# timoklein/alphazero-gym

Hardware: AMD Instinct MI355X
Metric: MCTS sims/sec (whole node), Pendulum-v1 4096 trees n_sims=200, 1/2/4/8 GPU (higher is better)
Workload: dtype f32; 1 GPU; config C: Pendulum-v1 A0C, 4096 trees/GPU x 200 sims, 2x256 ELU policy/value MLP, c_uct=0.05 c_pw=1 kappa=0.5; trees_per_gpu=4096, n_sims=200, parallelism=1 GPU

## Files before the change

### alphazero_gym_amd/csrc/azg_engine.hip

```cpp
#include <hip/hip_runtime.h>

#include <cmath>
#include <cstdio>
#include <cstdlib>
#include <cstring>
#include <string>
#include <vector>

#include "engine_host.h"
#include "env.cuh"
#include "mlp.cuh"
#include "tree.cuh"
#include "aux_kernels.cuh"


static std::string g_create_err;

static int fail(azg_engine* e, int code, const std::string& msg) {
    if (e) e->err = msg; else g_create_err = msg;
    return code;
}

#define HIPCHK(e, call)                                                                                  \
    do {                                                                                                 \
        hipError_t _rc = (call);                                                                         \
        if (_rc != hipSuccess) return fail(e, AZG_E_DEVICE, std::string(#call) + ": " + hipGetErrorString(_rc)); \
    } while (0)

struct DeviceScope {
    int prev;
    bool ok;
    explicit DeviceScope(int dev) : prev(-1) {
        if (hipGetDevice(&prev) != hipSuccess) prev = -1;
        ok = (prev == dev) || hipSetDevice(dev) == hipSuccess;
        if (prev == dev) prev = -1;
    }
    ~DeviceScope() { if (prev >= 0) (void)hipSetDevice(prev); }
};
#define ON_DEVICE(e)                                     \
    DeviceScope _scope((e)->cfg.device_id);              \
    if (!_scope.ok) return fail(e, AZG_E_DEVICE, "hipSetDevice failed")

template <typename T>
static int dalloc(azg_engine* e, T** p, size_t n, std::vector<void*>& reg) {
    void* q = nullptr;
    hipError_t rc = hipMalloc(&q, n * sizeof(T) > 0 ? n * sizeof(T) : 16);
    if (rc != hipSuccess) return fail(e, AZG_E_DEVICE, std::string("hipMalloc: ") + hipGetErrorString(rc));
    reg.push_back(q);
    *p = (T*)q;
    return AZG_OK;
}

static int ls_prepare(azg_engine* e) {
    if (e->ls_hp == e->HP) return AZG_OK;
    for (void* p : e->ls_allocs) (void)hipFree(p);
    e->ls_allocs.clear();
    const size_t B = e->cfg.n_trees, G = ((B + TREES_PER_WG - 1) / TREES_PER_WG + 3) / 4 * 4, HP = e->HP;
    float* obsT; float *a0, *a1, *parts; LsTree* tr; LsLane* ln;
    e->team_cnt_bytes = (((B + 31) / 32) * 8 * 32 + 32) * sizeof(unsigned);
    if (dalloc(e, &e->d_team_cnt, e->team_cnt_bytes / 4, e->ls_allocs) ||
        dalloc(e, &obsT, G * 64, e->ls_allocs) || dalloc(e, &a0, G * HP * 16, e->ls_allocs) || dalloc(e, &a1, G * HP * 16, e->ls_allocs) ||
        dalloc(e, &parts, G * (HP / 64) * 64 * 4, e->ls_allocs) || dalloc(e, &tr, B, e->ls_allocs) ||
        dalloc(e, &ln, B * 16, e->ls_allocs))
        return AZG_E_DEVICE;
    e->ls.obsT = obsT; e->ls.act[0] = (f32x4*)a0; e->ls.act[1] = (f32x4*)a1; e->ls.parts = (f32x4*)parts;
    e->ls.tree = tr; e->ls.lane = ln;
    if (hipMemset(obsT, 0, G * 64 * sizeof(float)) != hipSuccess || hipMemset(a0, 0, G * HP * 16 * sizeof(float)) != hipSuccess || hipMemset(a1, 0, G * HP * 16 * sizeof(float)) != hipSuccess) return AZG_E_DEVICE;
    e->ls_hp = e->HP;
    return AZG_OK;
}

static size_t stamp_rows(size_t B) {
    size_t r = ((B + 3) / 4) * 4;
    const size_t r8 = ((B + 15) / 16) * 8, team = ((B + 31) / 32) * 16 * 3 / 2;
    if (r8 > r) r = r8;
    if (team > r) r = team;
    return r < 16 ? 16 : r;
}

static int env_digit(const char* name, int dflt) {
    const char* v = getenv(name);
    return (v && v[0] >= '0' && v[0] <= '9') ? v[0] - '0' : dflt;
}

static bool use_lockstep(const azg_engine* e) {
    if (e->opt.force_persistent) return false;
    if (e->P.in8) return false;
    return e->HP >= 512 && e->n_hidden >= 2 && !e->P.layernorm;
}

template <int ENV>
static hipError_t search_path(azg_engine* e, bool lockstep) {
    if (lockstep) {
        if constexpr (ENV == AZG_ENV_ACROBOT) return hipErrorInvalidValue;
        else return azg_lockstep_search<ENV>(e);
    }
    return e->HP <= 128 ? azg_persistent_search<ENV, false>(e) : azg_persistent_search<ENV, true>(e);
}
static hipError_t search_launch(azg_engine* e, bool lockstep) {
    switch (azg_kernel_env(e->cfg)) {
        case AZG_ENV_CARTPOLE: return search_path<AZG_ENV_CARTPOLE>(e, lockstep);
        case AZG_ENV_MOUNTAINCAR_CONT: return search_path<AZG_ENV_MOUNTAINCAR_CONT>(e, lockstep);
        case AZG_ENV_ACROBOT: return search_path<AZG_ENV_ACROBOT>(e, lockstep);
        default: return search_path<AZG_ENV_PENDULUM_V1>(e, lockstep);
    }
}

extern "C" int azg_search_resident(azg_engine* e);
static int team_check(azg_engine* e) {
    if (!e->team_pending) return AZG_OK;
    unsigned flag = 0;
    e->team_pending = 0;
    if (hipMemcpy(&flag, e->d_team_cnt + (e->team_cnt_bytes / 4 - 1), 4, hipMemcpyDeviceToHost) != hipSuccess)
        return fail(e, AZG_E_DEVICE, "reading the team kernel's status failed");
    if (flag) e->opt.ls_team = 0;
    if (flag == 0) return AZG_OK;
    e->team_fallbacks += 1;
    e->search_idx = e->team_search_idx;
    int rc = azg_search_resident(e);
    if (rc) return rc;
    if (hipStreamSynchronize(e->stream) != hipSuccess) return fail(e, AZG_E_DEVICE, "hipStreamSynchronize failed");
    return AZG_OK;
}

extern "C" {

int azg_abi_version(void) { return AZG_ABI_VERSION; }

const char* azg_last_error(const azg_engine* e) { return e ? e->err.c_str() : g_create_err.c_str(); }

void azg_engine_destroy(azg_engine* e) {
    if (!e) return;
    DeviceScope scope(e->cfg.device_id);
    if (e->stream) (void)hipStreamSynchronize(e->stream);
    for (void* p : e->dev_allocs) (void)hipFree(p);
    for (void* p : e->dist_allocs) (void)hipFree(p);
    if (e->d_wblob) (void)hipFree(e->d_wblob);
    if (e->d_wmap) (void)hipFree(e->d_wmap);
    if (e->h_res_block) (void)hipHostFree(e->h_res_block);
    if (e->d_eval) (void)hipFree(e->d_eval);
    for (void* p : e->sp_allocs) (void)hipFree(p);
    for (void* p : e->ls_allocs) (void)hipFree(p);
    if (e->ev0) (void)hipEventDestroy(e->ev0);
    if (e->ev1) (void)hipEventDestroy(e->ev1);
    if (e->stream) (void)hipStreamDestroy(e->stream);
    delete e;
}

static int mapped_hip_runtimes(std::string& paths) {
    static int cached_n = -1;
    static std::string cached_paths;
    if (cached_n >= 0) { paths = cached_paths; return cached_n; }
    std::vector<std::string> seen;
    FILE* f = fopen("/proc/self/maps", "r");
    if (!f) return 0;
    char line[1024];
    while (fgets(line, sizeof line, f)) {
        if (!strstr(line, "libamdhip64")) continue;
        const char* p = strchr(line, '/');
        if (!p) continue;
        std::string path(p);
        while (!path.empty() && (path.back() == '\n' || path.back() == ' ')) path.pop_back();
        bool dup = false;
        for (const auto& q : seen) dup = dup || q == path;
        if (!dup) seen.push_back(path);
    }
    fclose(f);
    paths.clear();
    for (const auto& q : seen) paths += (paths.empty() ? "" : ", ") + q;
    cached_paths = paths;
    cached_n = (int)seen.size();
    return cached_n;
}

int azg_engine_create(const azg_config* cfg, azg_engine** out) {
    if (!cfg || !out) return fail(nullptr, AZG_E_INVALID, "null argument");
    {
        std::string rts;
        const char* allow = getenv("AZG_ALLOW_MULTI_HIP");
        if (mapped_hip_runtimes(rts) > 1 && !(allow && allow[0] == '1'))
            return fail(nullptr, AZG_E_DEVICE, ("two HIP runtimes are mapped in this process (" + rts + "): load PyTorch (import torch) BEFORE "
                                               "libazgym_hip.so so that both use PyTorch's copy; if they are meant to coexist (differing "
                                               "SONAMEs, a deliberate second copy), set AZG_ALLOW_MULTI_HIP=1").c_str());
    }
    if (cfg->struct_size != (int32_t)sizeof(azg_config)) return fail(nullptr, AZG_E_INVALID, "azg_config size mismatch");
    if (cfg->n_trees < 1 || cfg->n_sims < 1) return fail(nullptr, AZG_E_INVALID, "n_trees and n_sims must be >= 1");
    if (cfg->env_id < 0 || cfg->env_id > AZG_ENV_ACROBOT) return fail(nullptr, AZG_E_INVALID, "unknown env_id");
    const bool discrete_env = cfg->env_id == AZG_ENV_CARTPOLE || cfg->env_id == AZG_ENV_MOUNTAINCAR || cfg->env_id == AZG_ENV_ACROBOT;
    if (cfg->mode == AZG_MODE_DISCRETE && !discrete_env)
        return fail(nullptr, AZG_E_UNSUPPORTED, "discrete mode requires a discrete-action env (CartPole, MountainCar, Acrobot)");
    if (cfg->mode == AZG_MODE_CONTINUOUS && discrete_env)
        return fail(nullptr, AZG_E_UNSUPPORTED, "continuous mode requires a continuous-action env (Pendulum, MountainCarContinuous)");
    if (cfg->mode == AZG_MODE_DISCRETE && cfg->num_actions != (cfg->env_id == AZG_ENV_CARTPOLE ? 2 : 3))
        return fail(nullptr, AZG_E_INVALID, "num_actions does not match the env (CartPole 2, MountainCar 3, Acrobot 3)");
    if (cfg->tie_break != AZG_TIE_FIRST && cfg->tie_break != AZG_TIE_RANDOM) return fail(nullptr, AZG_E_INVALID, "unknown tie_break");
    if (cfg->mode == AZG_MODE_CONTINUOUS && !(cfg->c_pw > 0.0 && cfg->c_pw < 1e6 && cfg->kappa >= 0.0 && cfg->kappa <= 8.0))
        return fail(nullptr, AZG_E_INVALID, "c_pw must be > 0 and kappa >= 0 (progressive widening: ceil(c_pw (n + 1)^kappa) children)");
    int ndev = 0;
    if (hipGetDeviceCount(&ndev) != hipSuccess || ndev < 1) return fail(nullptr, AZG_E_DEVICE, "no HIP device available");
    if (cfg->device_id < 0 || cfg->device_id >= ndev) return fail(nullptr, AZG_E_DEVICE, "device_id out of range");
    azg_engine* e = new azg_engine();
    e->cfg = *cfg;
    e->opt.force_persistent = env_digit("AZG_FORCE_PERSISTENT", 0) == 1;
    e->opt.force_stream_weights = env_digit("AZG_FORCE_STREAM_WEIGHTS", 0) == 1;
    e->opt.force_global_tree = env_digit("AZG_FORCE_GLOBAL_TREE", 0) == 1;
    e->opt.no_spec = env_digit("AZG_NO_SPEC", 0) == 1;
    e->opt.waves = env_digit("AZG_WAVES", 0);
    e->opt.groups = env_digit("AZG_GROUPS", 0);
    { const char* v = getenv("AZG_TRACE_CAP"); const int t = v ? atoi(v) : 0; e->opt.trace_cap = t > 0 ? t : 0; }
    { const char* v = getenv("AZG_TILE_TREES"); const int t = v ? atoi(v) : 0; e->opt.tile_trees = (t == 16 || t == 8) ? t : 0; }
    e->opt.ls_team = env_digit("AZG_LS_TEAM", 1);
    e->opt.team_wide = env_digit("AZG_TEAM_WIDE", 1);
    { const char* v = getenv("AZG_TEAM_TT"); e->opt.team_tt = v ? atoi(v) : 0; }
    { const char* v = getenv("AZG_TEAM_SPIN_LIMIT"); e->opt.team_spin_limit = v ? atol(v) : (1L << 23); }
    e->opt.no_lds_state = getenv("AZG_NO_LDS_STATE") != nullptr;
    e->d_team_cnt = nullptr; e->team_cnt_bytes = 0; e->team_pending = 0; e->team_fallbacks = 0; e->team_search_idx = 0;
    e->lds_warned = 0; e->last_search_idx = 0; e->ms_kept = 0.0f; e->ms_kept_valid = 0;
    e->carry_max = 0;
    e->n_nets = 1; e->net_have.assign(1, 0);
    e->h_res_block = nullptr; e->d_res_block = nullptr; e->res_bytes = 0;
    e->d_wblob = nullptr; e->d_wmap = nullptr; e->w_floats = 0; e->dist_nd = -1; e->dist_ncomp = -1;
    e->d_eval = nullptr; e->eval_floats = 0;
    e->stream = nullptr; e->ev0 = e->ev1 = nullptr;
    e->publish_always = env_digit("AZG_PUBLISH_TREES", 0) == 1; e->publish_once = 0; e->published = 0; e->redo_ok = 0;
    e->mlp_ready = 0; e->searched = 0; e->results_valid = 0; e->search_idx = 0; e->last_ms = 0.0f; e->sp_on = 0; e->ls_hp = 0;
    e->S_env = (cfg->env_id == AZG_ENV_CARTPOLE || cfg->env_id == AZG_ENV_ACROBOT) ? 4 : 2;
    e->S_obs = cfg->env_id == AZG_ENV_ACROBOT ? 6 : (cfg->env_id == AZG_ENV_CARTPOLE ? 4 : ((cfg->env_id == AZG_ENV_MOUNTAINCAR || cfg->env_id == AZG_ENV_MOUNTAINCAR_CONT) ? 2 : 3));
    const int ns = cfg->n_sims;
    std::vector<int> pw(ns + 2, 0);
    if (cfg->mode == AZG_MODE_CONTINUOUS) {
        int kmax = 1;
        for (int n = 0; n < ns + 2; ++n) {
            double v = std::ceil(cfg->c_pw * std::pow((double)(n + 1), cfg->kappa));
            if (v > 1e6) v = 1e6;
            pw[n] = (int)v;
            if (n < ns && pw[n] > kmax) kmax = pw[n];
        }
        e->Kmax = kmax;
        e->R = ns + 2;
        e->nd = 2;
    } else {
        e->Kmax = cfg->num_actions;
        e->R = 1 + cfg->num_actions * (ns + 1);
        e->nd = cfg->num_actions;
    }
    if (e->R > 32767) { delete e; return fail(nullptr, AZG_E_UNSUPPORTED, "tree too large: records per tree must be < 32768"); }
    if (cfg->tie_break == AZG_TIE_RANDOM && e->Kmax > 16) { delete e; return fail(nullptr, AZG_E_UNSUPPORTED, "tie_break random supports at most 16 children per node"); }
    e->Kp = (e->Kmax + 15) / 16 * 16;
    e->tab_n = cfg->mode == AZG_MODE_CONTINUOUS ? ns + 2 : 4 * ns + 4;
    DeviceScope scope(cfg->device_id);
    if (!scope.ok) { delete e; return fail(nullptr, AZG_E_DEVICE, "hipSetDevice failed"); }
    e->n_cus = 256;
    (void)hipDeviceGetAttribute(&e->n_cus, hipDeviceAttributeMultiprocessorCount, cfg->device_id);
#define CK(x) do { int _r = (x); if (_r != AZG_OK) { g_create_err = e->err; azg_engine_destroy(e); return _r; } } while (0)
#define HK(call) do { hipError_t _rc = (call); if (_rc != hipSuccess) { g_create_err = std::string(#call) + ": " + hipGetErrorString(_rc); azg_engine_destroy(e); return AZG_E_DEVICE; } } while (0)
    HK(hipStreamCreateWithFlags(&e->stream, hipStreamNonBlocking));
    HK(hipEventCreate(&e->ev0));
    HK(hipEventCreate(&e->ev1));
    KParams& P = e->P;
    memset(&P, 0, sizeof(P));
    const size_t B = (size_t)cfg->n_trees, R = (size_t)e->R;
    RecL* hot; Cold* cold; double* edge_W; float* action; float* prior; unsigned short* child; int* n_rec;
    int* d_pw; double* d_sq;
    CK(dalloc(e, &hot, B * R, e->dev_allocs));
    CK(dalloc(e, &cold, B * R, e->dev_allocs));
    CK(dalloc(e, &edge_W, B * R, e->dev_allocs));
    CK(dalloc(e, &action, B * R, e->dev_allocs));
    CK(dalloc(e, &prior, B * R, e->dev_allocs));
    CK(dalloc(e, &child, B * R * e->Kp, e->dev_allocs));
    CK(dalloc(e, &n_rec, B, e->dev_allocs));
    CK(dalloc(e, &d_pw, (size_t)ns + 2, e->dev_allocs));
    CK(dalloc(e, &d_sq, (size_t)e->tab_n, e->dev_allocs));
    CK(dalloc(e, &e->d_roots, B * e->S_env, e->dev_allocs));
    CK(dalloc(e, &e->d_carry, B, e->dev_allocs));
    const size_t K = (size_t)e->Kmax;
    {
        e->res_bytes = B * K * 8 + B * 8 + B * K * 4 + B * K * 4 + B * 4;
        char* blk;
        CK(dalloc(e, &blk, e->res_bytes, e->dev_allocs));
        e->d_res_block = blk;
        e->d_Q = (double*)blk; e->d_vt = (double*)(blk + B * K * 8);
        e->d_actions = (float*)(blk + B * K * 8 + B * 8); e->d_counts = (int*)(blk + B * K * 8 + B * 8 + B * K * 4);
        e->d_nch = (int*)(blk + B * K * 8 + B * 8 + B * K * 8);
        HK(hipHostMalloc(&e->h_res_block, e->res_bytes, hipHostMallocDefault));
    }
    CK(dalloc(e, &e->d_child_n, B * K, e->dev_allocs));
    CK(dalloc(e, &e->d_child_state, B * K * e->S_env, e->dev_allocs));
    CK(dalloc(e, &e->d_rootV, B, e->dev_allocs));
    CK(dalloc(e, &e->d_rootdist, B * e->nd, e->dev_allocs));
    {
        unsigned long long* st;
        CK(dalloc(e, &st, stamp_rows(B) * 16, e->dev_allocs));
        e->P.stamps = st;
        e->stamp_n = stamp_rows(B);
    }
    std::vector<double> sq(e->tab_n);
    for (int n = 0; n < e->tab_n; ++n) sq[n] = std::sqrt((double)(n + 1));
    HK(hipMemcpy(d_pw, pw.data(), sizeof(int) * (ns + 2), hipMemcpyHostToDevice));
    HK(hipMemcpy(d_sq, sq.data(), sizeof(double) * e->tab_n, hipMemcpyHostToDevice));
    HK(hipMemset(hot, 0, B * R * sizeof(RecL)));
    HK(hipMemset(e->d_carry, 0, B * sizeof(int)));
    P.B = cfg->n_trees; P.n_sims = ns; P.R = e->R; P.Kp = e->Kp; P.A = cfg->num_actions; P.nd = e->nd;
    P.trace_cap = e->opt.trace_cap > 0 ? e->opt.trace_cap : 5;
    P.tie_random = cfg->tie_break == AZG_TIE_RANDOM; P.env_id = cfg->env_id; P.v1 = cfg->env_id == AZG_ENV_PENDULUM_V1; P.tree_base = cfg->tree_id_base; P.mode = cfg->mode;
    P.c_uct = cfg->c_uct; P.gamma = cfg->gamma; P.epsilon = cfg->epsilon; P.reward_scale = cfg->reward_scale;
    P.c_uct_f = (float)cfg->c_uct; P.gamma_f = (float)cfg->gamma; P.bound_f = (float)cfg->action_bound;
    P.seed = cfg->seed; P.S = e->S_env; P.tab_n = e->tab_n; P.pw0 = cfg->mode == AZG_MODE_CONTINUOUS ? pw[0] : 0;
    P.roots = e->d_roots; P.carry = e->d_carry;
    P.hot = hot; P.cold = cold; P.edge_W = edge_W; P.action = action; P.prior = prior; P.child = child;
    P.n_rec = n_rec; P.pw_need = d_pw; P.sqrt_tab = d_sq;
    P.res_actions = e->d_actions; P.res_counts = e->d_counts; P.res_Q = e->d_Q; P.res_vt = e->d_vt; P.res_nch = e->d_nch;
    P.res_child_n = e->d_child_n; P.res_child_state = e->d_child_state; P.res_root_V = e->d_rootV; P.res_root_dist = e->d_rootdist;
    P.res_Kmax = e->Kmax; P.res_v_target = cfg->v_target;
    P.net_T = cfg->n_trees; P.net_wgs = 1; P.net_wstride = 0;
    *out = e;
    return AZG_OK;
#undef CK
#undef HK
}

static int pad64(int n) { return (n + 63) / 64 * 64; }
static inline int unit_of(int i) { int t = i >> 4, r = (i >> 2) & 3, g = i & 3; return 16 * t + 4 * g + r; }

static bool same_desc(const azg_mlp_desc& a, const azg_mlp_desc& b) {
    if (a.in_dim != b.in_dim || a.n_hidden != b.n_hidden || a.n_dist != b.n_dist || a.layernorm != b.layernorm) return false;
    for (int l = 0; l < a.n_hidden; ++l) if (a.hidden[l] != b.hidden[l]) return false;
    return true;
}

static int check_desc(azg_engine* e, const azg_mlp_desc* d, size_t n_floats, int* HP_out, int* ncomp_out) {
    if (d->struct_size != (int32_t)sizeof(azg_mlp_desc)) return fail(e, AZG_E_INVALID, "azg_mlp_desc size mismatch");
    if (d->n_hidden < 1 || d->n_hidden > AZG_MAX_HIDDEN_LAYERS) return fail(e, AZG_E_INVALID, "n_hidden out of range");
    if (d->activation < 0 || d->activation > AZG_ACT_HARDSWISH) return fail(e, AZG_E_INVALID, "unknown activation");
    if (d->in_dim != e->S_obs) return fail(e, AZG_E_INVALID, "in_dim does not match the env observation");
    int ncomp = 0;
    if (e->cfg.mode == AZG_MODE_CONTINUOUS) {
        ncomp = d->num_components >= 2 ? d->num_components : 0;
        if (ncomp > 5) return fail(e, AZG_E_UNSUPPORTED, "at most 5 mixture components");
        if (d->n_dist != (ncomp ? 3 * ncomp : 2)) return fail(e, AZG_E_INVALID, "n_dist does not match num_components");
    } else if (d->n_dist != e->nd) return fail(e, AZG_E_INVALID, "n_dist does not match the engine mode");
    if (1 + d->n_dist > 16) return fail(e, AZG_E_UNSUPPORTED, "at most 15 distribution outputs");
    size_t need = 0;
    int k = d->in_dim, hmax = 0;
    for (int l = 0; l < d->n_hidden; ++l) {
        if (d->hidden[l] < 1 || d->hidden[l] > 4096) return fail(e, AZG_E_INVALID, "hidden width out of range");
        need += (size_t)d->hidden[l] * k + d->hidden[l] + (d->layernorm ? 2 * (size_t)d->hidden[l] : 0);
        k = d->hidden[l];
        if (k > hmax) hmax = k;
    }
    need += (size_t)(1 + d->n_dist) * k + (1 + d->n_dist);
    if (need != n_floats) return fail(e, AZG_E_INVALID, "weight blob size mismatch");
    const int HP = pad64(hmax);
    if (HP != 64 && HP != 128 && HP != 256 && HP != 512 && HP != 1024)
        return fail(e, AZG_E_UNSUPPORTED, "hidden width (padded to a multiple of 64) must be one of 64,128,256,512,1024");
    *HP_out = HP;
    *ncomp_out = ncomp;
    return AZG_OK;
}

static void build_weight_map(const azg_mlp_desc* d, int HP, WeightMap& m) {
    typedef unsigned idx_t;
    const int NT = HP / 16, S4 = HP / 16;
    std::vector<std::vector<idx_t>> Wd(d->n_hidden), bd(d->n_hidden), gd(d->n_hidden), ed(d->n_hidden);
    idx_t p = 1;
    const int kp0 = d->in_dim > 4 ? 8 : 4;
    int kt = d->in_dim, kp = kp0;
    for (int l = 0; l < d->n_hidden; ++l) {
        const int h = d->hidden[l];
        Wd[l].assign((size_t)HP * kp, 0);
        bd[l].assign(HP, 0);
        for (int n = 0; n < h; ++n)
            for (int kk = 0; kk < kt; ++kk) Wd[l][(size_t)n * kp + kk] = p + (idx_t)((size_t)n * kt + kk);
        p += (idx_t)((size_t)h * kt);
        for (int n = 0; n < h; ++n) bd[l][n] = p + n;
        p += h;
        gd[l].assign(HP, 0);
        ed[l].assign(HP, 0);
        if (d->layernorm) {
            for (int n = 0; n < h; ++n) gd[l][n] = p + n;
            p += h;
            for (int n = 0; n < h; ++n) ed[l][n] = p + n;
            p += h;
        }
        kt = h; kp = HP;
    }
    std::vector<idx_t> Wh((size_t)16 * HP, 0), bh(16, 0);
    for (int kk = 0; kk < kt; ++kk) Wh[kk] = p + kk;
    p += kt;
    bh[0] = p++;
    for (int o = 0; o < d->n_dist; ++o)
        for (int kk = 0; kk < kt; ++kk) Wh[(size_t)(1 + o) * HP + kk] = p + (idx_t)((size_t)o * kt + kk);
    p += (idx_t)((size_t)d->n_dist * kt);
    for (int o = 0; o < d->n_dist; ++o) bh[1 + o] = p + o;
    std::vector<idx_t>& st = m.src;
    st.clear();
    auto reserve = [&](size_t n) { size_t off = st.size(); st.resize(off + (n + 63) / 64 * 64, 0); return off; };
    m.oW0 = reserve((size_t)NT * 64); m.ob0 = reserve((size_t)NT * 64 * 4);
    m.oW0b = reserve((size_t)NT * 64);
    for (int t = 0; t < NT; ++t)
        for (int l = 0; l < 64; ++l) {
            const int row = 16 * t + (l & 15), g = l >> 4;
            st[m.oW0 + (size_t)t * 64 + l] = Wd[0][(size_t)row * kp0 + g];
            st[m.oW0b + (size_t)t * 64 + l] = kp0 == 8 ? Wd[0][(size_t)row * kp0 + 4 + g] : 0;
            for (int r = 0; r < 4; ++r) st[m.ob0 + ((size_t)t * 64 + l) * 4 + r] = bd[0][16 * t + 4 * g + r];
        }
    m.oW0u = reserve((size_t)HP * 4); m.ob0u = reserve((size_t)HP);
    for (int u = 0; u < HP; ++u) {
        for (int kk = 0; kk < 4; ++kk) st[m.oW0u + (size_t)u * 4 + kk] = Wd[0][(size_t)u * kp0 + kk];
        st[m.ob0u + u] = bd[0][u];
    }
    for (int l = 0; l < MAX_STREAM_LAYERS; ++l) { m.oWl[l] = m.obl[l] = m.olg[l] = m.olb[l] = 0; }
    for (int l = 1; l < d->n_hidden; ++l) {
        const size_t oW = reserve((size_t)NT * S4 * 64 * 4), ob = reserve((size_t)NT * 64 * 4);
        m.oWl[l - 1] = oW; m.obl[l - 1] = ob;
        for (int t = 0; t < NT; ++t)
            for (int l64 = 0; l64 < 64; ++l64) {
                const int row = 16 * t + (l64 & 15), g = l64 >> 4;
                for (int s4 = 0; s4 < S4; ++s4)
                    for (int j = 0; j < 4; ++j) {
                        const int i = 4 * (4 * s4 + j) + g;
                        st[oW + (((size_t)t * S4 + s4) * 64 + l64) * 4 + j] = Wd[l][(size_t)row * HP + unit_of(i)];
                    }
                for (int r = 0; r < 4; ++r) st[ob + ((size_t)t * 64 + l64) * 4 + r] = bd[l][16 * t + 4 * g + r];
            }
    }
    m.oWh = reserve((size_t)S4 * 64 * 4); m.obh = reserve(16);
    for (int s4 = 0; s4 < S4; ++s4)
        for (int l64 = 0; l64 < 64; ++l64) {
            const int o = l64 & 15, g = l64 >> 4;
            for (int j = 0; j < 4; ++j) {
                const int i = 4 * (4 * s4 + j) + g;
                st[m.oWh + ((size_t)s4 * 64 + l64) * 4 + j] = Wh[(size_t)o * HP + unit_of(i)];
            }
        }
    for (int o = 0; o < 16; ++o) st[m.obh + o] = bh[o];
    if (d->layernorm)
        for (int l = 0; l < d->n_hidden; ++l) {
            m.olg[l] = reserve((size_t)NT * 64 * 4); m.olb[l] = reserve((size_t)NT * 64 * 4);
            for (int t = 0; t < NT; ++t)
                for (int l64 = 0; l64 < 64; ++l64)
                    for (int r = 0; r < 4; ++r) {
                        st[m.olg[l] + ((size_t)t * 64 + l64) * 4 + r] = gd[l][16 * t + 4 * (l64 >> 4) + r];
                        st[m.olb[l] + ((size_t)t * 64 + l64) * 4 + r] = ed[l][16 * t + 4 * (l64 >> 4) + r];
                    }
        }
    m.desc = *d;
    m.HP = HP;
    m.valid = true;
}

__global__ __launch_bounds__(256) void weight_gather_kernel(const unsigned* __restrict__ src, const float* __restrict__ blob,
                                                            float* __restrict__ out, size_t n) {
    const size_t i = (size_t)blockIdx.x * 256 + threadIdx.x;
    if (i < n) { const unsigned s = src[i]; out[i] = s ? blob[s - 1] : 0.0f; }
}

__global__ __launch_bounds__(256) void weight_gather_nets_kernel(const unsigned* __restrict__ src, const float* __restrict__ blob,
                                                                 size_t blob_stride, float* __restrict__ out, size_t n) {
    const size_t i = (size_t)blockIdx.x * 256 + threadIdx.x;
    const size_t k = blockIdx.y;
    if (i < n) { const unsigned s = src[i]; out[k * n + i] = s ? blob[k * blob_stride + s - 1] : 0.0f; }
}

static int set_weights_impl(azg_engine* e, const azg_mlp_desc* d, const float* blob, size_t n_floats, bool on_device, int net = 0,
                            int n_write = 1) {
    if (!e || !d || !blob) return AZG_E_INVALID;
    if (n_write != 1 && !on_device) return AZG_E_INVALID;
    int HP = 0, ncomp = 0;
    { int rc = check_desc(e, d, n_floats, &HP, &ncomp); if (rc) return rc; }
    const int NN = e->n_nets;
    bool others = false;
    for (int k = 0; k < NN; ++k) others = others || ((k < net || k >= net + n_write) && e->net_have[k]);
    if (NN > 1) {
        if (HP >= 512)
            return fail(e, AZG_E_UNSUPPORTED, "populations: networks wider than 256 (padded) run as team / per-layer searches, which take one "
                                              "network per engine");
        if (others && !(e->wmap.valid && e->wmap.HP == HP && same_desc(e->wmap.desc, *d) && d->activation == e->wmap.desc.activation &&
                        d->num_components == e->wmap.desc.num_components && d->log_std_min == e->wmap.desc.log_std_min &&
                        d->log_std_max == e->wmap.desc.log_std_max))
            return fail(e, AZG_E_INVALID, "populations: every net must have the same network descriptor (azg_mlp_desc)");
    }
    ON_DEVICE(e);
    HIPCHK(e, hipStreamSynchronize(e->stream));
    { int trc = team_check(e); if (trc) return trc; }
    e->mlp_ready = 0;
    e->results_valid = 0;
    e->redo_ok = 0;
    WeightMap& m = e->wmap;
    if (!m.valid || m.HP != HP || !same_desc(m.desc, *d)) {
        m.valid = false;
        build_weight_map(d, HP, m);
        if (e->d_wmap) { (void)hipFree(e->d_wmap); e->d_wmap = nullptr; }
    }
    m.desc = *d;
    const size_t n_out_f = m.src.size();
    if (n_out_f != e->w_floats || !e->d_wblob) {
        if (e->d_wblob) (void)hipFree(e->d_wblob);
        e->d_wblob = nullptr; e->w_floats = 0;
        for (int k = 0; k < NN; ++k) e->net_have[k] = 0;
        void* q = nullptr;
        HIPCHK(e, hipMalloc(&q, n_out_f * NN * sizeof(float)));
        e->d_wblob = (float*)q; e->w_floats = n_out_f;
    }
    float* const wnet = e->d_wblob + (size_t)net * n_out_f;
    for (int k = net; k < net + n_write; ++k) e->net_have[k] = 0;
    if (on_device) {
        if (!e->d_wmap) {
            void* q = nullptr;
            HIPCHK(e, hipMalloc(&q, n_out_f * sizeof(unsigned)));
            e->d_wmap = (unsigned*)q;
            HIPCHK(e, hipMemcpy(e->d_wmap, m.src.data(), n_out_f * sizeof(unsigned), hipMemcpyHostToDevice));
        }
        if (n_write == 1)
            hipLaunchKernelGGL(weight_gather_kernel, dim3((unsigned)((n_out_f + 255) / 256)), dim3(256), 0, e->stream, e->d_wmap, blob, wnet, n_out_f);
        else
            for (int k0 = 0; k0 < n_write; k0 += 65535) {
                const int nk = n_write - k0 < 65535 ? n_write - k0 : 65535;
                hipLaunchKernelGGL(weight_gather_nets_kernel, dim3((unsigned)((n_out_f + 255) / 256), (unsigned)nk), dim3(256), 0, e->stream,
                                   e->d_wmap, blob + (size_t)k0 * n_floats, n_floats, wnet + (size_t)k0 * n_out_f, n_out_f);
            }
        HIPCHK(e, hipGetLastError());
        HIPCHK(e, hipStreamSynchronize(e->stream));
    } else {
        std::vector<float>& st = e->w_stage;
        st.resize(n_out_f);
        const unsigned* src = m.src.data();
        for (size_t i = 0; i < n_out_f; ++i) st[i] = src[i] ? blob[src[i] - 1] : 0.0f;
        HIPCHK(e, hipMemcpy(wnet, st.data(), n_out_f * sizeof(float), hipMemcpyHostToDevice));
    }
    for (int k = net; k < net + n_write; ++k) e->net_have[k] = 1;
    e->P.net_wstride = NN > 1 ? n_out_f : 0;
    const float* wb = e->d_wblob;
    e->P.W0u = (const f32x4*)(wb + m.oW0u);
    e->P.b0u = (const f32x4*)(wb + m.ob0u);
    e->P.W0 = wb + m.oW0;
    e->P.W0b = wb + m.oW0b;
    e->P.in8 = d->in_dim > 4 ? 1 : 0;
    e->P.b0 = (const f32x4*)(wb + m.ob0);
    for (int l = 0; l < MAX_STREAM_LAYERS; ++l) {
        const bool on = l + 1 < d->n_hidden;
        e->P.Wl[l] = on ? (const f32x4*)(wb + m.oWl[l]) : nullptr;
        e->P.bl[l] = on ? (const f32x4*)(wb + m.obl[l]) : nullptr;
    }
    e->P.Whead = (const f32x4*)(wb + m.oWh);
    e->P.bhead = wb + m.obh;
    e->P.layernorm = d->layernorm ? 1 : 0;
    for (int l = 0; l < MAX_STREAM_LAYERS; ++l) {
        e->P.Htrue[l] = l < d->n_hidden ? d->hidden[l] : 0;
        e->P.lng[l] = (d->layernorm && l < d->n_hidden) ? (const f32x4*)(wb + m.olg[l]) : nullptr;
        e->P.lnb[l] = (d->layernorm && l < d->n_hidden) ? (const f32x4*)(wb + m.olb[l]) : nullptr;
    }
    if (e->cfg.mode == AZG_MODE_CONTINUOUS && (d->n_dist != e->dist_nd || ncomp != e->dist_ncomp)) {
        for (void* q : e->dist_allocs) (void)hipFree(q);
        e->dist_allocs.clear();
        e->dist_nd = -1; e->searched = 0;
        float* g = nullptr;
        if (ncomp) { if (dalloc(e, &g, (size_t)e->cfg.n_trees * e->R * 3 * GMM_MAXC, e->dist_allocs)) return AZG_E_DEVICE; }
        float* rd = nullptr;
        if (dalloc(e, &rd, (size_t)e->cfg.n_trees * d->n_dist, e->dist_allocs)) return AZG_E_DEVICE;
        e->P.gmm = g; e->P.ncomp = ncomp; e->d_rootdist = rd; e->P.res_root_dist = rd; e->nd = d->n_dist; e->P.nd = d->n_dist;
        e->dist_nd = d->n_dist; e->dist_ncomp = ncomp;
    }
    const int n_out = 1 + d->n_dist;
    e->HP = HP; e->n_hidden = d->n_hidden; e->n_out = n_out; e->act = d->activation;
    e->P.n_hidden = d->n_hidden; e->P.n_out = n_out; e->P.act = d->activation; e->P.ls_min = d->log_std_min; e->P.ls_max = d->log_std_max;
    int nhh = d->n_hidden - 1;
    int regs = nhh * (HP * HP / 256);
    e->nreg = (nhh >= 1 && nhh <= 2 && regs <= 288) ? nhh : 0;
    if (d->layernorm || (d->activation != AZG_ACT_RELU && d->activation != AZG_ACT_ELU)) e->nreg = 0;
    if (e->opt.force_stream_weights) e->nreg = 0;
    bool all = true;
    for (int k = 0; k < NN; ++k) all = all && e->net_have[k];
    e->mlp_ready = all ? 1 : 0;
    return AZG_OK;
}

static const char* kPopWeights = "this engine holds a population (azg_set_population > 1): upload each net's weights with azg_set_net_weights";

int azg_set_weights(azg_engine* e, const azg_mlp_desc* d, const float* blob, size_t n_floats) {
    if (e && e->n_nets > 1) return fail(e, AZG_E_STATE, kPopWeights);
    return set_weights_impl(e, d, blob, n_floats, false);
}

int azg_set_weights_device(azg_engine* e, const azg_mlp_desc* d, const float* device_blob, size_t n_floats) {
    if (e && e->n_nets > 1) return fail(e, AZG_E_STATE, kPopWeights);
    return set_weights_impl(e, d, device_blob, n_floats, true);
}

int azg_set_population(azg_engine* e, int32_t n_nets) {
    if (!e) return AZG_E_INVALID;
    if (n_nets < 1 || n_nets > e->cfg.n_trees || e->cfg.n_trees % n_nets != 0)
        return fail(e, AZG_E_INVALID, "azg_set_population: n_nets must divide n_trees (trees k*T .. k*T+T-1 belong to net k, T = n_trees / n_nets)");
    if (e->sp_on) return fail(e, AZG_E_UNSUPPORTED, "azg_set_population: device self-play is running on this engine (one network per engine)");
    if (n_nets == e->n_nets) return AZG_OK;
    ON_DEVICE(e);
    HIPCHK(e, hipStreamSynchronize(e->stream));
    { int trc = team_check(e); if (trc) return trc; }
    const size_t rows = stamp_rows((size_t)n_nets * (((size_t)e->cfg.n_trees / n_nets + 15) / 16 * 16));
    if (rows > e->stamp_n) {
        unsigned long long* st = nullptr;
        if (dalloc(e, &st, rows * 16, e->dev_allocs)) return AZG_E_DEVICE;
        for (size_t i = 0; i < e->dev_allocs.size(); ++i)
            if (e->dev_allocs[i] == (void*)e->P.stamps) { (void)hipFree(e->dev_allocs[i]); e->dev_allocs.erase(e->dev_allocs.begin() + i); break; }
        e->P.stamps = st; e->stamp_n = rows;
    }
    if (e->d_wblob) (void)hipFree(e->d_wblob);
    e->d_wblob = nullptr; e->w_floats = 0;
    e->n_nets = n_nets;
    e->net_have.assign(n_nets, 0);
    e->mlp_ready = 0; e->results_valid = 0; e->redo_ok = 0; e->searched = 0;
    e->P.net_T = e->cfg.n_trees / n_nets; e->P.net_wstride = 0;
    return AZG_OK;
}

int azg_set_net_weights(azg_engine* e, int32_t net, const azg_mlp_desc* d, const float* blob, size_t n_floats) {
    if (!e) return AZG_E_INVALID;
    if (net < 0 || net >= e->n_nets) return fail(e, AZG_E_INVALID, "azg_set_net_weights: net index out of range");
    return set_weights_impl(e, d, blob, n_floats, false, net);
}

int azg_set_net_weights_device(azg_engine* e, int32_t net, const azg_mlp_desc* d, const float* device_blob, size_t n_floats) {
    if (!e) return AZG_E_INVALID;
    if (net < 0 || net >= e->n_nets) return fail(e, AZG_E_INVALID, "azg_set_net_weights_device: net index out of range");
    return set_weights_impl(e, d, device_blob, n_floats, true, net);
}

int azg_set_population_weights_device(azg_engine* e, const azg_mlp_desc* d, const float* device_blobs, size_t n_floats_per_net, int32_t n_nets) {
    if (!e) return AZG_E_INVALID;
    if (n_nets != e->n_nets)
        return fail(e, AZG_E_INVALID, "azg_set_population_weights_device: n_nets must equal the engine's number of nets (azg_set_population)");
    return set_weights_impl(e, d, device_blobs, n_floats_per_net, true, 0, n_nets);
}

int azg_set_search_index(azg_engine* e, uint32_t idx) { if (!e) return AZG_E_INVALID; e->search_idx = idx; return AZG_OK; }

int azg_upload_roots(azg_engine* e, const double* roots, const int32_t* carry) {
    if (!e || !roots) return AZG_E_INVALID;
    const int B = e->cfg.n_trees, S = e->S_env;
    if (e->cfg.env_id == AZG_ENV_CARTPOLE) {
        const double theta_thr = 12.0 * 2.0 * 3.141592653589793 / 360.0, x_thr = 2.4;
        for (int i = 0; i < B; ++i) {
            const double* s = roots + (size_t)i * S;
            if ((s[0] < -x_thr) || (s[0] > x_thr) || (s[2] < -theta_thr) || (s[2] > theta_thr))
                return fail(e, AZG_E_TERMINAL_ROOT, "Can't do tree search from a terminal node");
        }
    } else if (e->cfg.env_id == AZG_ENV_ACROBOT) {
        for (int i = 0; i < B; ++i)
            if (azg_acrobot_terminal(roots + (size_t)i * S)) return fail(e, AZG_E_TERMINAL_ROOT, "Can't do tree search from a terminal node");
    } else if (e->cfg.env_id == AZG_ENV_MOUNTAINCAR || e->cfg.env_id == AZG_ENV_MOUNTAINCAR_CONT) {
        const double goal = e->cfg.env_id == AZG_ENV_MOUNTAINCAR ? 0.5 : 0.45;
        for (int i = 0; i < B; ++i) {
            const double* s = roots + (size_t)i * S;
            if (s[0] >= goal && s[1] >= 0.0) return fail(e, AZG_E_TERMINAL_ROOT, "Can't do tree search from a terminal node");
        }
    }
    int cmax = 0;
    if (carry)
        for (int i = 0; i < B; ++i) {
            if (carry[i] < 0 || carry[i] > (1 << 30)) return fail(e, AZG_E_INVALID, "root_n_carry out of range");
            if (carry[i] != 0 && e->cfg.mode == AZG_MODE_CONTINUOUS)
                return fail(e, AZG_E_INVALID, "root_n_carry: continuous searches start from a fresh root (no carried count)");
            if (carry[i] > cmax) cmax = carry[i];
        }
    ON_DEVICE(e);
    if (e->team_pending) {
        HIPCHK(e, hipStreamSynchronize(e->stream));
        int trc = team_check(e);
        if (trc) return trc;
    }
    e->carry_max = cmax;
    e->redo_ok = 0;
    HIPCHK(e, hipMemcpyAsync(e->d_roots, roots, sizeof(double) * (size_t)B * S, hipMemcpyHostToDevice, e->stream));
    if (carry) HIPCHK(e, hipMemcpyAsync(e->d_carry, carry, sizeof(int) * (size_t)B, hipMemcpyHostToDevice, e->stream));
    else HIPCHK(e, hipMemsetAsync(e->d_carry, 0, sizeof(int) * (size_t)B, e->stream));
    HIPCHK(e, hipStreamSynchronize(e->stream));
    return AZG_OK;
}

int azg_search_resident(azg_engine* e) {
    if (!e) return AZG_E_INVALID;
    if (!e->mlp_ready)
        return fail(e, AZG_E_STATE, e->n_nets > 1 ? "azg_set_net_weights has not been called for every net of the population"
                                                 : "azg_set_weights has not been called");
    if (e->n_nets > 1 && use_lockstep(e))
        return fail(e, AZG_E_UNSUPPORTED, "populations run on the one-launch search kernel only");
    ON_DEVICE(e);
    e->P.search_idx = e->search_idx;
    e->last_search_idx = e->search_idx;
    e->ms_kept_valid = 0;
    e->P.publish = (e->publish_always || e->publish_once) ? 1 : 0;
    e->team_search_idx = e->search_idx;
    e->last = LaunchRecord();
    const bool lockstep = use_lockstep(e);
    if (lockstep) { int prc = ls_prepare(e); if (prc) return prc; }
    if (lockstep) HIPCHK(e, hipEventRecord(e->ev0, e->stream));
    const hipError_t rc = search_launch(e, lockstep);
    if (rc != hipSuccess) return fail(e, AZG_E_DEVICE, std::string("search kernel launch: ") + hipGetErrorString(rc));
    if (!e->last.timed) HIPCHK(e, hipEventRecord(e->ev1, e->stream));
    e->search_idx += 1;
    e->searched = 1;
    const bool persistent = e->last.form == AZG_FORM_PERSISTENT;
    e->results_valid = persistent ? 1 : 0;
    e->published = (!persistent || e->last.tree_lds == TS_GLOBAL || e->P.publish) ? 1 : 0;
    e->redo_ok = 1;
    if (persistent && e->last.tree_lds == TS_GLOBAL && e->last.lds_exit != AZG_LDS_EXIT_FORCED && !e->lds_warned) {
        e->lds_warned = 1;
        static const char* why[] = {"", "more than 511 records per tree (n_sims + 2)", "more than 16 children per node (c_pw / kappa)",
                                    "the workgroup's LDS plan exceeds the CU's 160 KB", "", "",
                                    "the root's visit count (carried + n_sims) overflows the LDS records' counters"};
        const int x = e->last.lds_exit;
        const char* reason = x == AZG_LDS_EXIT_RECORDS && e->R <= 511 ? "more than 255 records per tree (n_sims + 2) for this network's kernels"
                                                                      : (x >= 0 && x < (int)(sizeof(why) / sizeof(why[0])) ? why[x] : "");
        if (!getenv("AZG_QUIET"))
            fprintf(stderr, "azgym: the trees of this search do not fit LDS residency (%s): they are kept in global memory -- same results, "
                            "slower tree walk (azg_search_info; once per engine)\n", reason);
    }
    return AZG_OK;
}

int azg_sync(azg_engine* e) {
    if (!e) return AZG_E_INVALID;
    ON_DEVICE(e);
    HIPCHK(e, hipStreamSynchronize(e->stream));
    return team_check(e);
}

int azg_search(azg_engine* e, const double* roots, const int32_t* carry) {
    int rc = azg_upload_roots(e, roots, carry);
    if (rc) return rc;
    rc = azg_search_resident(e);
    if (rc) return rc;
    return azg_sync(e);
}

int azg_last_search_ms(azg_engine* e, float* ms) {
    if (!e || !ms) return AZG_E_INVALID;
    if (!e->searched) return fail(e, AZG_E_STATE, "no search has run");
    ON_DEVICE(e);
    HIPCHK(e, hipEventSynchronize(e->ev1));
    if (e->team_pending) {
        HIPCHK(e, hipStreamSynchronize(e->stream));
        int trc = team_check(e);
        if (trc) return trc;
    }
    if (e->ms_kept_valid) { *ms = e->ms_kept; return AZG_OK; }
    HIPCHK(e, hipEventElapsedTime(ms, e->ev0, e->ev1));
    return AZG_OK;
}

static int launch_results(azg_engine* e) {
    if (!e->searched) return fail(e, AZG_E_STATE, "no search has run");
    if (e->results_valid) return AZG_OK;
    if (e->team_pending) {
        HIPCHK(e, hipStreamSynchronize(e->stream));
        int trc = team_check(e);
        if (trc) return trc;
    }
    int B = e->cfg.n_trees;
    hipLaunchKernelGGL(results_kernel, dim3((B + RS_TREES - 1) / RS_TREES), dim3(16 * RS_TREES), 0, e->stream, e->P);
    HIPCHK(e, hipGetLastError());
    e->results_valid = 1;
    return AZG_OK;
}

static int gather_results(azg_engine* e) {
    ON_DEVICE(e);
    int rc = launch_results(e);
    if (rc) return rc;
    HIPCHK(e, hipStreamSynchronize(e->stream));
    return AZG_OK;
}

#define D2H(dst, src, bytes) do { if (dst) HIPCHK(e, hipMemcpy(dst, src, bytes, hipMemcpyDeviceToHost)); } while (0)

int azg_results(azg_engine* e, float* actions, int32_t* counts, double* Q, double* v_target, int32_t* n_children) {
    if (!e) return AZG_E_INVALID;
    ON_DEVICE(e);
    int rc = launch_results(e);
    if (rc) return rc;
    const size_t B = e->cfg.n_trees, K = e->Kmax;
    HIPCHK(e, hipMemcpyAsync(e->h_res_block, e->d_res_block, e->res_bytes, hipMemcpyDeviceToHost, e->stream));
    HIPCHK(e, hipStreamSynchronize(e->stream));
    const char* h = (const char*)e->h_res_block;
    if (Q) memcpy(Q, h, B * K * 8);
    if (v_target) memcpy(v_target, h + B * K * 8, B * 8);
    if (actions) memcpy(actions, h + B * K * 8 + B * 8, B * K * 4);
    if (counts) memcpy(counts, h + B * K * 8 + B * 8 + B * K * 4, B * K * 4);
    if (n_children) memcpy(n_children, h + B * K * 8 + B * 8 + B * K * 8, B * 4);
    return AZG_OK;
}

int azg_results_resident(azg_engine* e, const float** actions, const int32_t** counts, const double** Q, const double** v_target,
                         const int32_t** n_children) {
    if (!e) return AZG_E_INVALID;
    ON_DEVICE(e);
    int rc = launch_results(e);
    if (rc) return rc;
    if (actions) *actions = e->d_actions;
    if (counts) *counts = e->d_counts;
    if (Q) *Q = e->d_Q;
    if (v_target) *v_target = e->d_vt;
    if (n_children) *n_children = e->d_nch;
    return AZG_OK;
}

int azg_root_children(azg_engine* e, int32_t* child_n, double* child_state) {
    if (!e) return AZG_E_INVALID;
    int rc = gather_results(e);
    if (rc) return rc;
    size_t B = e->cfg.n_trees, K = e->Kmax;
    D2H(child_n, e->d_child_n, B * K * 4);
    D2H(child_state, e->d_child_state, B * K * e->S_env * 8);
    return AZG_OK;
}

int azg_root_eval(azg_engine* e, float* value, float* dist) {
    if (!e) return AZG_E_INVALID;
    if (e->n_nets > 1) return fail(e, AZG_E_UNSUPPORTED, "azg_root_eval: not available for populations (azg_set_population > 1)");
    int rc = gather_results(e);
    if (rc) return rc;
    size_t B = e->cfg.n_trees;
    D2H(value, e->d_rootV, B * 4);
    D2H(dist, e->d_rootdist, B * e->nd * 4);
    return AZG_OK;
}

int azg_mlp_eval(azg_engine* e, const float* obs, size_t n, float* value, float* dist, float* raw) {
    if (!e || !obs) return AZG_E_INVALID;
    if (e->n_nets > 1) return fail(e, AZG_E_UNSUPPORTED, "azg_mlp_eval: not available for populations (azg_set_population > 1): evaluate each net's policy");
    if (!e->mlp_ready) return fail(e, AZG_E_STATE, "azg_set_weights has not been called");
    if (n == 0) return AZG_OK;
    if (n > (size_t)1 << 24) return fail(e, AZG_E_INVALID, "too many observations in one call");
    ON_DEVICE(e);
    const size_t So = e->S_obs, nd = e->nd;
    const size_t need = n * (So + 1 + nd + 1 + nd);
    if (need > e->eval_floats) {
        if (e->d_eval) (void)hipFree(e->d_eval);
        e->d_eval = nullptr; e->eval_floats = 0;
        void* q = nullptr;
        HIPCHK(e, hipMalloc(&q, need * sizeof(float)));
        e->d_eval = (float*)q; e->eval_floats = need;
    }
    float* d_obs = e->d_eval;
    float* d_v = d_obs + n * So;
    float* d_d = d_v + n;
    float* d_r = d_d + n * nd;
    HIPCHK(e, hipMemcpyAsync(d_obs, obs, n * So * 4, hipMemcpyHostToDevice, e->stream));
    hipError_t rc = azg_dispatch_mlp_eval(e, d_obs, (int)n, d_v, d_d, d_r);
    if (rc != hipSuccess) return fail(e, AZG_E_DEVICE, std::string("mlp_eval kernel launch: ") + hipGetErrorString(rc));
    HIPCHK(e, hipStreamSynchronize(e->stream));
    D2H(value, d_v, n * 4);
    D2H(dist, d_d, n * nd * 4);
    D2H(raw, d_r, n * (nd + 1) * 4);
    return AZG_OK;
}

int azg_dump_tree(azg_engine* e, int32_t* n_records, int32_t* parent, int32_t* edge_n, double* edge_W, double* edge_Q,
                  float* edge_action, int32_t* node_n, double* node_r, float* node_V, uint8_t* node_flags) {
    if (!e) return AZG_E_INVALID;
    if (!e->searched) return fail(e, AZG_E_STATE, "no search has run");
    ON_DEVICE(e);
    HIPCHK(e, hipStreamSynchronize(e->stream));
    { int trc = team_check(e); if (trc) return trc; }
    if (!e->published) {
        if (!e->redo_ok)
            return fail(e, AZG_E_STATE, "the last search's trees were not written out and its inputs have changed since (self-play step, new "
                                        "roots or weights): dump right after the search, or set AZG_PUBLISH_TREES=1");
        float ms_before = 0.0f;
        HIPCHK(e, hipEventElapsedTime(&ms_before, e->ev0, e->ev1));
        const uint32_t idx_now = e->search_idx;
        e->publish_once = 1;
        e->search_idx = e->last_search_idx;
        int rc = azg_search_resident(e);
        e->publish_once = 0;
        e->search_idx = idx_now;
        if (rc) return rc;
        HIPCHK(e, hipStreamSynchronize(e->stream));
        { int trc = team_check(e); if (trc) return trc; }
        e->ms_kept = ms_before; e->ms_kept_valid = 1;
    }
    size_t B = e->cfg.n_trees, R = e->R;
    std::vector<RecL> hot(B * R);
    std::vector<Cold> cold(B * R);
    std::vector<int> nrec(B);
    std::vector<double> ew(B * R);
    std::vector<float> ac(B * R);
    HIPCHK(e, hipMemcpy(hot.data(), e->P.hot, B * R * sizeof(RecL), hipMemcpyDeviceToHost));
    HIPCHK(e, hipMemcpy(cold.data(), e->P.cold, B * R * sizeof(Cold), hipMemcpyDeviceToHost));
    HIPCHK(e, hipMemcpy(nrec.data(), e->P.n_rec, B * 4, hipMemcpyDeviceToHost));
    HIPCHK(e, hipMemcpy(ew.data(), e->P.edge_W, B * R * 8, hipMemcpyDeviceToHost));
    HIPCHK(e, hipMemcpy(ac.data(), e->P.action, B * R * 4, hipMemcpyDeviceToHost));
    const bool cont = e->cfg.mode == AZG_MODE_CONTINUOUS;
    const int A = e->cfg.num_actions;
    for (size_t i = 0; i < B; ++i) {
        if (n_records) n_records[i] = nrec[i];
        for (size_t j = 0; j < R; ++j) {
            size_t o = i * R + j;
            bool in = (int)j < nrec[i];
            const RecL& h = hot[o];
            bool ex = in && (h.flags & FLAG_EXPANDED);
            if (parent) parent[o] = in ? (j == 0 ? -1 : h.parent) : 0;
            if (edge_n) edge_n[o] = in ? h.edge_n : 0;
            if (edge_W) edge_W[o] = in ? ew[o] : 0.0;
            if (edge_Q) edge_Q[o] = in ? h.Q : 0.0;
            if (edge_action) edge_action[o] = in ? (cont ? ac[o] : (j == 0 ? 0.0f : (float)((j - 1) % A))) : 0.0f;
            if (node_n) node_n[o] = in ? h.node_n : 0;
            if (node_r) node_r[o] = ex ? cold[o].r : 0.0;
            if (node_V) node_V[o] = ex ? cold[o].V : 0.0f;
            if (node_flags) node_flags[o] = in ? h.flags : 0;
        }
    }
    return AZG_OK;
}

static int kernel_name(const azg_engine* e, char* buf, size_t n) {
    const int env = azg_kernel_env(e->cfg);
    const char* gmm = (env != AZG_ENV_CARTPOLE && e->P.ncomp >= 2) ? "true" : "false";
    const LaunchRecord& r = e->last;
    switch (r.form) {
        case AZG_FORM_PERSISTENT: return snprintf(buf, n, "search_kernel<%d, %d, %d, %d, %s, %d, %d, %d, %d>", env, e->HP, e->nreg, r.tree_lds, gmm, r.waves, r.groups, r.tile_trees, r.spec);
        case AZG_FORM_PER_LAYER: return snprintf(buf, n, "ls_tree_kernel<%d, ...> + ls_layer0_kernel + ls_hidden_tiled_kernel<%d, ...> per simulation step", env, e->HP);
        case AZG_FORM_TEAM: return snprintf(buf, n, "ls_team_kernel<%d, %d, %s, %d, %d, %d, %d, %d>", env, e->HP, gmm, r.tree_lds, r.team_kc, r.team_minb, r.spec, r.team_tt);
        default: return snprintf(buf, n, "(no search yet)");
    }
}

int azg_search_info(azg_engine* e, azg_search_report* info) {
    if (!e || !info) return AZG_E_INVALID;
    if (info->struct_size != (int32_t)sizeof(azg_search_report)) return fail(e, AZG_E_INVALID, "azg_search_info: struct_size mismatch");
    if (e->searched && e->team_pending) {
        ON_DEVICE(e);
        HIPCHK(e, hipStreamSynchronize(e->stream));
        int trc = team_check(e);
        if (trc) return trc;
    }
    memset(info, 0, sizeof(*info));
    info->struct_size = (int32_t)sizeof(azg_search_report);
    const LaunchRecord& r = e->last;
    info->kernel_form = e->searched ? r.form : AZG_FORM_NONE;
    info->max_records = e->R; info->max_children = e->Kmax;
    info->team_fallbacks = e->team_fallbacks;
    if (!e->searched) { kernel_name(e, info->kernel_name, sizeof(info->kernel_name)); info->lds_exit = AZG_LDS_RESIDENT; return AZG_OK; }
    info->tree_storage = r.form == AZG_FORM_PERSISTENT ? r.tree_lds : AZG_TREES_GLOBAL;
    info->lds_exit = r.lds_exit;
    info->spec = r.spec;
    info->waves = r.waves; info->groups = r.groups; info->tile_trees = r.tile_trees;
    if (r.form == AZG_FORM_TEAM) { info->team_trees = r.team_tt; info->team_per_cu = r.team_minb; info->team_parts = r.team_parts; }
    float ms = 0.0f;
    int rc = azg_last_search_ms(e, &ms);
    if (rc) return rc;
    info->last_ms = ms;
    kernel_name(e, info->kernel_name, sizeof(info->kernel_name));
    return AZG_OK;
}

int azg_debug_stamps(azg_engine* e, unsigned long long* out, size_t max_rows) {
    if (!e || !out) return AZG_E_INVALID;
    size_t rows = e->stamp_n;
    if (rows > max_rows) rows = max_rows;
    ON_DEVICE(e);
    HIPCHK(e, hipStreamSynchronize(e->stream));
    HIPCHK(e, hipMemcpy(out, e->P.stamps, rows * 16 * sizeof(unsigned long long), hipMemcpyDeviceToHost));
    return (int)rows;
}

int azg_max_children(const azg_engine* e) { return e ? e->Kmax : AZG_E_INVALID; }
int azg_max_records(const azg_engine* e) { return e ? e->R : AZG_E_INVALID; }
int azg_env_state_dim(const azg_engine* e) { return e ? e->S_env : AZG_E_INVALID; }
int azg_obs_dim(const azg_engine* e) { return e ? e->S_obs : AZG_E_INVALID; }

int azg_synthetic_roots(azg_engine* e, double* roots) {
    if (!e || !roots) return AZG_E_INVALID;
    for (int i = 0; i < e->cfg.n_trees; ++i)
        azg_reset_state(e->cfg.seed, (uint32_t)(e->cfg.tree_id_base + i), 0u, azg_reset_kind(e->cfg.env_id), roots + (size_t)i * e->S_env);
    return AZG_OK;
}

int azg_selfplay_row_len(const azg_engine* e) { return e ? e->S_obs + 3 * e->Kmax + 1 : AZG_E_INVALID; }

static int selfplay_begin_impl(azg_engine* e, const azg_selfplay_config* c) {
    if (c->struct_size != (int32_t)sizeof(azg_selfplay_config)) return fail(e, AZG_E_INVALID, "azg_selfplay_config size mismatch");
    if (c->max_episode_length < 1 || c->capacity_steps < 1) return fail(e, AZG_E_INVALID, "max_episode_length and capacity_steps must be >= 1");
    if (c->final_selection != AZG_FS_MAX_VISIT && c->final_selection != AZG_FS_MAX_VALUE) return fail(e, AZG_E_INVALID, "unknown final_selection");
    if (c->ring_mode != AZG_RING_STOP && c->ring_mode != AZG_RING_FIFO) return fail(e, AZG_E_INVALID, "unknown ring_mode");
    if (!(c->temperature > 0.0)) return fail(e, AZG_E_INVALID, "temperature must be > 0");
    if (c->agent_epsilon < 0.0 || c->agent_epsilon > 1.0) return fail(e, AZG_E_INVALID, "agent_epsilon must be in [0, 1]");
    const bool discrete = e->cfg.mode == AZG_MODE_DISCRETE;
    if (discrete && c->final_selection == AZG_FS_MAX_VALUE && c->temperature != 1.0)
        return fail(e, AZG_E_UNSUPPORTED, "final_selection max_value on the device supports temperature 1 only");
    ON_DEVICE(e);
    HIPCHK(e, hipStreamSynchronize(e->stream));
    for (void* p : e->sp_allocs) (void)hipFree(p);
    e->sp_allocs.clear();
    e->sp_on = 0;
    const size_t B = e->cfg.n_trees;
    e->sp_row = e->S_obs + 3 * e->Kmax + 1;
    if (dalloc(e, &e->d_sp_t, B, e->sp_allocs) || dalloc(e, &e->d_sp_episode, B, e->sp_allocs) || dalloc(e, &e->d_sp_fcnt, B, e->sp_allocs) ||
        dalloc(e, &e->d_sp_ret, B, e->sp_allocs) || dalloc(e, &e->d_sp_fsum, B, e->sp_allocs) ||
        dalloc(e, &e->d_sp_rows, (size_t)c->capacity_steps * B * e->sp_row, e->sp_allocs))
        return AZG_E_DEVICE;
    e->d_sp_ctab = nullptr;
    if (discrete && c->temperature != 1.0) {
        const size_t ns = (size_t)e->cfg.n_sims;
        if (ns > 2048) return fail(e, AZG_E_UNSUPPORTED, "temperature != 1 on the device supports n_sims <= 2048");
        std::vector<double> tab((ns + 1) * (ns + 2) / 2, 0.0);
        for (size_t m = 1; m <= ns; ++m)
            for (size_t k = 0; k <= m; ++k) tab[m * (m + 1) / 2 + k] = std::pow((double)k / (double)m, c->temperature);
        if (dalloc(e, &e->d_sp_ctab, tab.size(), e->sp_allocs)) return AZG_E_DEVICE;
        HIPCHK(e, hipMemcpy(e->d_sp_ctab, tab.data(), tab.size() * 8, hipMemcpyHostToDevice));
    }
    HIPCHK(e, hipMemset(e->d_sp_t, 0, B * 4));
    HIPCHK(e, hipMemset(e->d_sp_episode, 0, B * 4));
    HIPCHK(e, hipMemset(e->d_sp_fcnt, 0, B * 4));
    HIPCHK(e, hipMemset(e->d_sp_ret, 0, B * 8));
    HIPCHK(e, hipMemset(e->d_sp_fsum, 0, B * 8));
    std::vector<double> roots(B * e->S_env);
    azg_synthetic_roots(e, roots.data());
    HIPCHK(e, hipMemcpy(e->d_roots, roots.data(), roots.size() * 8, hipMemcpyHostToDevice));
    HIPCHK(e, hipMemset(e->d_carry, 0, B * 4));
    e->carry_max = discrete ? e->cfg.n_sims : 0;
    e->sp_on = 1; e->sp_max_len = c->max_episode_length; e->sp_det = c->deterministic; e->sp_cap = c->capacity_steps; e->sp_steps = 0;
    e->sp_insert = 0; e->sp_total = 0; e->sp_fs = c->final_selection; e->sp_ring = c->ring_mode; e->sp_agent_eps = c->agent_epsilon;
    e->sp_step_idx = 0;
    return AZG_OK;
}

int azg_selfplay_begin_ex(azg_engine* e, const azg_selfplay_config* c) {
    if (!e || !c) return AZG_E_INVALID;
    if (e->n_nets > 1)
        return fail(e, AZG_E_UNSUPPORTED, "device self-play of a population (azg_set_population > 1) starts with azg_population_selfplay_begin");
    return selfplay_begin_impl(e, c);
}

int azg_population_selfplay_begin(azg_engine* e, const azg_selfplay_config* c) {
    if (!e || !c) return AZG_E_INVALID;
    return selfplay_begin_impl(e, c);
}

int azg_selfplay_begin(azg_engine* e, int32_t max_episode_length, int32_t deterministic, int32_t capacity_steps) {
    azg_selfplay_config c;
    memset(&c, 0, sizeof(c));
    c.struct_size = (int32_t)sizeof(c);
    c.max_episode_length = max_episode_length; c.deterministic = deterministic; c.capacity_steps = capacity_steps;
    c.final_selection = AZG_FS_MAX_VISIT; c.ring_mode = AZG_RING_STOP; c.temperature = 1.0; c.agent_epsilon = 0.0;
    return azg_selfplay_begin_ex(e, &c);
}

int azg_selfplay_step(azg_engine* e) {
    if (!e) return AZG_E_INVALID;
    if (!e->sp_on) return fail(e, AZG_E_STATE, "azg_selfplay_begin has not been called");
    if (e->sp_ring == AZG_RING_STOP && e->sp_steps >= e->sp_cap) return fail(e, AZG_E_STATE, "replay ring is full: download and clear the rows");
    int rc = azg_search_resident(e);
    if (rc) return rc;
    ON_DEVICE(e);
    if (e->team_pending) {
        HIPCHK(e, hipStreamSynchronize(e->stream));
        rc = team_check(e);
        if (rc) return rc;
    }
    int slot;
    if (e->sp_steps < e->sp_cap) { slot = e->sp_steps; e->sp_steps += 1; }
    else { slot = e->sp_insert; e->sp_insert = (e->sp_insert + 1) % e->sp_steps; }
    SelfPlay sp;
    sp.max_len = e->sp_max_len; sp.deterministic = e->sp_det; sp.step_idx = e->sp_step_idx;
    sp.final_selection = e->sp_fs; sp.agent_eps = e->sp_agent_eps; sp.ctab = e->d_sp_ctab;
    sp.t = e->d_sp_t; sp.episode = e->d_sp_episode; sp.fcnt = e->d_sp_fcnt; sp.ret = e->d_sp_ret; sp.fsum = e->d_sp_fsum;
    sp.rows = e->d_sp_rows + (size_t)slot * e->cfg.n_trees * e->sp_row;
    sp.roots = e->d_roots; sp.carry = e->d_carry;
    const int B = e->cfg.n_trees;
    e->redo_ok = 0;
    if (e->Kmax <= 16) {
        rc = launch_results(e);
        if (rc) return rc;
    }
    if (e->Kmax <= 16)
        hipLaunchKernelGGL(selfplay_kernel16, dim3((B + SP_TREES - 1) / SP_TREES), dim3(16 * SP_TREES), 0, e->stream, e->P, sp, e->Kmax, e->cfg.v_target, e->cfg.env_id, e->S_obs);
    else
        hipLaunchKernelGGL(selfplay_kernel, dim3((B + RK_THREADS - 1) / RK_THREADS), dim3(RK_THREADS), 0, e->stream, e->P, sp, e->Kmax, e->cfg.v_target, e->cfg.env_id, e->S_obs);
    HIPCHK(e, hipGetLastError());
    e->sp_total += 1;
    e->sp_step_idx += 1;
    return AZG_OK;
}

int azg_selfplay_rows(azg_engine* e, float* rows, size_t max_rows, int32_t clear) {
    if (!e) return AZG_E_INVALID;
    if (!e->sp_on) return fail(e, AZG_E_STATE, "azg_selfplay_begin has not been called");
    ON_DEVICE(e);
    HIPCHK(e, hipStreamSynchronize(e->stream));
    size_t n = (size_t)e->sp_steps * e->cfg.n_trees;
    if (n > max_rows) n = max_rows;
    if (rows && n) HIPCHK(e, hipMemcpy(rows, e->d_sp_rows, n * e->sp_row * 4, hipMemcpyDeviceToHost));
    if (clear) { e->sp_steps = 0; e->sp_insert = 0; }
    return (int)n;
}

int azg_selfplay_ring(azg_engine* e, int32_t* size_steps, int32_t* insert_step, int64_t* total_steps) {
    if (!e) return AZG_E_INVALID;
    if (!e->sp_on) return fail(e, AZG_E_STATE, "azg_selfplay_begin has not been called");
    if (size_steps) *size_steps = e->sp_steps;
    if (insert_step) *insert_step = e->sp_insert;
    if (total_steps) *total_steps = e->sp_total;
    return AZG_OK;
}

int azg_selfplay_rows_device(azg_engine* e, void** device_ptr, size_t* capacity_rows, size_t* row_len) {
    if (!e || !device_ptr) return AZG_E_INVALID;
    if (!e->sp_on) return fail(e, AZG_E_STATE, "azg_selfplay_begin has not been called");
    *device_ptr = e->d_sp_rows;
    if (capacity_rows) *capacity_rows = (size_t)e->sp_cap * e->cfg.n_trees;
    if (row_len) *row_len = (size_t)e->sp_row;
    return AZG_OK;
}

int azg_selfplay_stats(azg_engine* e, double* fsum, int32_t* fcnt, double* env_state) {
    if (!e) return AZG_E_INVALID;
    if (!e->sp_on) return fail(e, AZG_E_STATE, "azg_selfplay_begin has not been called");
    ON_DEVICE(e);
    HIPCHK(e, hipStreamSynchronize(e->stream));
    size_t B = e->cfg.n_trees;
    D2H(fsum, e->d_sp_fsum, B * 8);
    D2H(fcnt, e->d_sp_fcnt, B * 4);
    D2H(env_state, e->d_roots, B * e->S_env * 8);
    return AZG_OK;
}

int azg_math_selftest(int device_id, int fn_id, const double* in, double* out, size_t n) {
    if (!in || !out || n == 0) return AZG_E_INVALID;
    DeviceScope scope(device_id);
    if (!scope.ok) return AZG_E_DEVICE;
    double *di = nullptr, *dout = nullptr;
    if (hipMalloc((void**)&di, n * 8) != hipSuccess) return AZG_E_DEVICE;
    if (hipMalloc((void**)&dout, n * 8) != hipSuccess) { (void)hipFree(di); return AZG_E_DEVICE; }
    int rc = AZG_OK;
    if (hipMemcpy(di, in, n * 8, hipMemcpyHostToDevice) != hipSuccess) rc = AZG_E_DEVICE;
    if (rc == AZG_OK) {
        if (fn_id == 100) {
            int K = (int)((n - 1) / 2);
            hipLaunchKernelGGL(mfma_probe_kernel, dim3(1), dim3(64), 0, 0, di, dout, K);
        } else if (fn_id == 102 && n >= 16) {
            int* chase = nullptr;
            std::vector<int> hc(1 << 16);
            for (size_t i = 0; i < hc.size(); ++i) hc[i] = (int)((i * 4099 + 77) & (hc.size() - 1));
            if (hipMalloc((void**)&chase, hc.size() * 4) == hipSuccess) {
                (void)hipMemcpy(chase, hc.data(), hc.size() * 4, hipMemcpyHostToDevice);
                hipLaunchKernelGGL(latency_probe_kernel, dim3(1), dim3(64), 0, 0, dout, chase, 4096);
                (void)hipDeviceSynchronize();
                (void)hipFree(chase);
            }
        } else if (fn_id == 101 && n >= 8) {
            const int wgs = (int)in[0], iters = (int)in[1], reps = (int)in[2] > 0 ? (int)in[2] : 1;
            hipEvent_t e0, e1;
            (void)hipEventCreate(&e0); (void)hipEventCreate(&e1);
            hipLaunchKernelGGL(mfma_rate_kernel, dim3(wgs), dim3(256), 0, 0, dout, iters);
            (void)hipEventRecord(e0, 0);
            for (int r = 0; r < reps; ++r) hipLaunchKernelGGL(mfma_rate_kernel, dim3(wgs), dim3(256), 0, 0, dout, iters);
            (void)hipEventRecord(e1, 0);
            (void)hipEventSynchronize(e1);
            float ms = 0.0f;
            (void)hipEventElapsedTime(&ms, e0, e1);
            double res[2] = {ms / reps, (double)wgs * 4 * iters * 16 * 2048.0 / (ms / reps * 1e-3) / 1e12};
            (void)hipMemcpy(dout + 3, res, sizeof(res), hipMemcpyHostToDevice);
            (void)hipEventDestroy(e0); (void)hipEventDestroy(e1);
        } else {
            hipLaunchKernelGGL(math_selftest_kernel, dim3((unsigned)((n + 255) / 256)), dim3(256), 0, 0, fn_id, di, dout, n);
        }
        if (hipGetLastError() != hipSuccess || hipDeviceSynchronize() != hipSuccess) rc = AZG_E_DEVICE;
    }
    if (rc == AZG_OK && hipMemcpy(out, dout, n * 8, hipMemcpyDeviceToHost) != hipSuccess) rc = AZG_E_DEVICE;
    (void)hipFree(di);
    (void)hipFree(dout);
    return rc;
}

}
```

### alphazero_gym_amd/csrc/dispatch.cuh

```cuda
#pragma once
#include <hip/hip_ext.h>

#include "engine_host.h"
#include "env.cuh"
#include "mlp.cuh"
#include "tree.cuh"
#include "search_kernel.cuh"

template <int ENV, int HP, int NREG, int TLDS, bool GMM, int NW, int NG, int NT = 16, int SPEC = 0>
static hipError_t launch_g(azg_engine* e) {
    auto kern = search_kernel<ENV, HP, NREG, TLDS, GMM, NW, NG, NT, SPEC>;
    static KernelAttrs attrs;
    int static_lds = 0;
    hipError_t rc = attrs.static_bytes((const void*)kern, &static_lds);
    if (rc != hipSuccess) return rc;
    constexpr bool CONT = EnvFamily<ENV>::CONT;
    const LdsLayout with_state = lds_layout(e->tab_n, e->cfg.n_sims, HP, NG, act_buffers(NREG), e->R, CONT, TLDS, 1, NT);
    const LdsLayout without = lds_layout(e->tab_n, e->cfg.n_sims, HP, NG, act_buffers(NREG), e->R, CONT, TLDS, 0, NT);
    const long n_wg = azg_padded_trees(e, NT * NG) / (NT * NG);
    const size_t room = 160 * 1024 - (size_t)static_lds;
    const bool costs_a_neighbour = n_wg > e->n_cus && 2 * (without.total + static_lds) <= 160 * 1024 && 2 * (with_state.total + static_lds) > 160 * 1024;
    e->P.lds_state = (!CONT && TLDS != TS_GLOBAL && with_state.total <= room && !costs_a_neighbour && !e->opt.no_lds_state) ? 1 : 0;
    const size_t lds = e->P.lds_state ? with_state.total : without.total;
    if (lds > room) return hipErrorInvalidConfiguration;
    rc = attrs.set_dyn_lds(e, (const void*)kern, lds);
    if (rc != hipSuccess) return rc;
    dim3 grid((unsigned)n_wg), block(64 * NW);
    e->P.net_wgs = (int)(n_wg / e->n_nets);
    LaunchRecord& r = e->last;
    r.form = AZG_FORM_PERSISTENT; r.tree_lds = TLDS; r.spec = SPEC;
    r.waves = NW; r.groups = NG; r.tile_trees = NT;
    hipExtLaunchKernelGGL(kern, grid, block, (unsigned)lds, e->stream, e->ev0, e->ev1, 0, e->P);
    r.timed = 1;
    return hipGetLastError();
}

template <int ENV, int HP, int NREG, int TLDS, int NW, int NG, int NT = 16>
static hipError_t launch_t(azg_engine* e) {
    if constexpr (EnvFamily<ENV>::CONT && NW == 4 && NT == 16 && TLDS != TS_LDS9) {
        if (e->P.ncomp >= 2) return launch_g<ENV, HP, NREG, TLDS, true, NW, NG>(e);
    }
    if constexpr (NREG == 1 && TLDS == TS_LDS8 && NT == 16 && ENV != AZG_ENV_ACROBOT) {
        const bool common = e->cfg.epsilon == 0.0 && e->cfg.tie_break == AZG_TIE_FIRST &&
                            (ENV != AZG_ENV_PENDULUM_V1 || e->cfg.env_id == AZG_ENV_PENDULUM_V1) &&
                            (ENV != AZG_ENV_CARTPOLE || (e->cfg.env_id == AZG_ENV_CARTPOLE && e->cfg.num_actions == 2 &&
                                                         (long)e->carry_max + e->cfg.n_sims + 2 <= (long)e->tab_n));
        if (common && !e->opt.no_spec) return launch_g<ENV, HP, NREG, TLDS, false, NW, NG, NT, 1>(e);
    }
    return launch_g<ENV, HP, NREG, TLDS, false, NW, NG, NT>(e);
}

template <int ENV, int HP, int NREG>
static hipError_t launch(azg_engine* e) {
    const TreeStorage st = azg_tree_storage(e, HP < 512 && e->P.ncomp < 2);
    const int ts = st.ts;
    e->last.lds_exit = st.lds_exit;
    if constexpr (HP == 256 && NREG == 1 && EnvFamily<ENV>::CONT) {
        bool two = azg_padded_trees(e, 16) / 16 > e->n_cus;
        if (e->opt.groups == 2) two = true;
        if (e->opt.groups == 1) two = false;
        bool want8 = true;
        if (e->opt.waves == 4) want8 = false;
        if (want8 && ts == TS_LDS8 && e->P.ncomp < 2) {
            hipError_t rc = hipErrorInvalidConfiguration;
            if (two) rc = launch_t<ENV, HP, NREG, TS_LDS8, 8, 2>(e);
            if (rc == hipErrorInvalidConfiguration) rc = launch_t<ENV, HP, NREG, TS_LDS8, 8, 1>(e);
            if (rc != hipErrorInvalidConfiguration) return rc;
        }
    }
    if constexpr (HP <= 128 && NREG == 1) {
        if (ts == TS_LDS8 && e->P.ncomp < 2) {
            int nt = azg_padded_trees(e, 8) <= 8L * e->n_cus ? 8 : 16;
            if (e->opt.tile_trees) nt = e->opt.tile_trees;
            if (nt == 8) {
                hipError_t rc = launch_t<ENV, HP, NREG, TS_LDS8, 4, 1, 8>(e);
                if (rc != hipErrorInvalidConfiguration) return rc;
            }
        }
    }
    if (ts == TS_LDS8) {
        hipError_t rc = launch_t<ENV, HP, NREG, TS_LDS8, 4, 1>(e);
        if (rc != hipErrorInvalidConfiguration) return rc;
    }
    if constexpr (HP < 512) {
        if (ts == TS_LDS9) {
            hipError_t rc = launch_t<ENV, HP, NREG, TS_LDS9, 4, 1>(e);
            if (rc != hipErrorInvalidConfiguration) return rc;
        }
    }
    if (ts != TS_GLOBAL) e->last.lds_exit = AZG_LDS_EXIT_SIZE;
    return launch_t<ENV, HP, NREG, TS_GLOBAL, 4, 1>(e);
}

template <int ENV, bool WIDE>
hipError_t azg_persistent_search(azg_engine* e) {
    const int HP = e->HP, NR = e->nreg;
    if constexpr (!WIDE) {
        if (HP == 64) return NR == 1 ? launch<ENV, 64, 1>(e) : NR == 2 ? launch<ENV, 64, 2>(e) : launch<ENV, 64, 0>(e);
        if (HP == 128) return NR == 1 ? launch<ENV, 128, 1>(e) : NR == 2 ? launch<ENV, 128, 2>(e) : launch<ENV, 128, 0>(e);
    } else {
        if (HP == 256) return NR == 1 ? launch<ENV, 256, 1>(e) : launch<ENV, 256, 0>(e);
        if (HP == 512) return launch<ENV, 512, 0>(e);
        if (HP == 1024) return launch<ENV, 1024, 0>(e);
    }
    return hipErrorInvalidValue;
}
```

### alphazero_gym_amd/csrc/engine_host.h

```cpp
#pragma once
#include <hip/hip_runtime.h>

#include <atomic>
#include <string>
#include <vector>

#include "records.h"
#include "../../include/azgym_population.h"

struct EngineOptions {
    int force_persistent;
    int force_stream_weights;
    int force_global_tree;
    int waves;
    int groups;
    int trace_cap;
    int no_spec;
    int tile_trees;
    int ls_team;
    int team_wide;
    int team_tt;
    long team_spin_limit;
    int no_lds_state;
};
#define AZG_MAX_DEVICES 64

struct LaunchRecord {
    int form = AZG_FORM_NONE;
    int tree_lds = TS_GLOBAL, spec = 0;
    int lds_exit = AZG_LDS_NOT_APPLICABLE;
    int waves = 0, groups = 0, tile_trees = 0;
    int team_kc = 0, team_minb = 0, team_tt = 0, team_parts = 0;
    int timed = 0;
};

struct WeightMap {
    bool valid = false;
    azg_mlp_desc desc;
    int HP = 0;
    std::vector<unsigned> src;
    size_t oW0, oW0b, ob0, oW0u, ob0u, oWl[MAX_STREAM_LAYERS], obl[MAX_STREAM_LAYERS], oWh, obh, olg[MAX_STREAM_LAYERS], olb[MAX_STREAM_LAYERS];
};

struct azg_engine {
    azg_config cfg;
    EngineOptions opt;
    int carry_max;
    int S_env, S_obs, Kmax, Kp, R, nd, tab_n;
    int mlp_ready, HP, n_hidden, n_out, act, nreg;
    int n_cus;
    LaunchRecord last;
    float ls_min, ls_max;
    hipStream_t stream;
    hipEvent_t ev0, ev1;
    KParams P;
    std::vector<void*> dev_allocs;
    float* d_wblob;
    size_t w_floats;
    std::vector<float> w_stage;
    WeightMap wmap;
    unsigned* d_wmap;
    std::vector<void*> dist_allocs;
    int dist_nd, dist_ncomp;
    float* d_actions; int* d_counts; double* d_Q; double* d_vt; int* d_nch; int* d_child_n; double* d_child_state;
    float* d_rootV; float* d_rootdist;
    char* d_res_block; void* h_res_block; size_t res_bytes;
    double* d_roots; int* d_carry;
    uint32_t search_idx;
    int sp_on, sp_max_len, sp_det, sp_cap, sp_steps, sp_row;
    int sp_insert, sp_fs, sp_ring;
    long long sp_total;
    double sp_agent_eps;
    double* d_sp_ctab;
    uint32_t sp_step_idx;
    int* d_sp_t; int* d_sp_episode; int* d_sp_fcnt; double* d_sp_ret; double* d_sp_fsum; float* d_sp_rows;
    std::vector<void*> sp_allocs;
    unsigned* d_team_cnt; size_t team_cnt_bytes;
    int team_pending;
    int team_fallbacks;
    uint32_t team_search_idx;
    int lds_warned;
    LockStep ls;
    std::vector<void*> ls_allocs;
    int ls_hp;
    float* d_eval; size_t eval_floats;
    int searched, results_valid;
    int publish_always;
    int publish_once;
    int published;
    int redo_ok;
    int n_nets;
    std::vector<char> net_have;
    size_t stamp_n;
    float last_ms;
    uint32_t last_search_idx;
    float ms_kept; int ms_kept_valid;
    std::string err;
};

static inline long azg_padded_trees(const azg_engine* e, int tpw) {
    const long T = e->cfg.n_trees / e->n_nets;
    return (long)e->n_nets * ((T + tpw - 1) / tpw * tpw);
}

static inline int azg_kernel_env(const azg_config& c) {
    if (c.mode == AZG_MODE_DISCRETE) return c.env_id == AZG_ENV_ACROBOT ? AZG_ENV_ACROBOT : AZG_ENV_CARTPOLE;
    return c.env_id == AZG_ENV_MOUNTAINCAR_CONT ? AZG_ENV_MOUNTAINCAR_CONT : AZG_ENV_PENDULUM_V1;
}

struct TreeStorage { int ts, lds_exit; };
static inline TreeStorage azg_tree_storage(const azg_engine* e, bool lds9) {
    const long nmax = (long)e->carry_max + e->cfg.n_sims + 2;
    if (e->opt.force_global_tree) return {TS_GLOBAL, AZG_LDS_EXIT_FORCED};
    if (e->Kp != 16) return {TS_GLOBAL, AZG_LDS_EXIT_CHILDREN};
    if (e->R <= 255) return nmax < 65536 ? TreeStorage{TS_LDS8, AZG_LDS_RESIDENT} : TreeStorage{TS_GLOBAL, AZG_LDS_EXIT_COUNTS};
    if (e->R > 511 || !lds9) return {TS_GLOBAL, AZG_LDS_EXIT_RECORDS};
    return nmax < 2048 ? TreeStorage{TS_LDS9, AZG_LDS_RESIDENT} : TreeStorage{TS_GLOBAL, AZG_LDS_EXIT_COUNTS};
}

struct KernelAttrs {
    std::atomic<int> static_lds{-1};
    std::atomic<size_t> dyn_lds[AZG_MAX_DEVICES] = {};
    std::atomic<int> per_cu[AZG_MAX_DEVICES] = {};

    hipError_t static_bytes(const void* kern, int* bytes) {
        if ((*bytes = static_lds.load(std::memory_order_relaxed)) >= 0) return hipSuccess;
        hipFuncAttributes fa;
        hipError_t rc = hipFuncGetAttributes(&fa, kern);
        if (rc == hipSuccess) static_lds.store(*bytes = (int)fa.sharedSizeBytes, std::memory_order_relaxed);
        return rc;
    }
    hipError_t set_dyn_lds(const azg_engine* e, const void* kern, size_t bytes) {
        std::atomic<size_t>& last = dyn_lds[e->cfg.device_id % AZG_MAX_DEVICES];
        if (last.load(std::memory_order_relaxed) == bytes) return hipSuccess;
        hipError_t rc = hipFuncSetAttribute(kern, hipFuncAttributeMaxDynamicSharedMemorySize, (int)bytes);
        if (rc == hipSuccess) last.store(bytes, std::memory_order_relaxed);
        return rc;
    }
    hipError_t occupancy(const azg_engine* e, const void* kern, int threads, size_t bytes, int* blocks) {
        std::atomic<int>& cached = per_cu[e->cfg.device_id % AZG_MAX_DEVICES];
        *blocks = cached.load(std::memory_order_relaxed);
        if (*blocks > 0 && dyn_lds[e->cfg.device_id % AZG_MAX_DEVICES].load(std::memory_order_relaxed) == bytes) return hipSuccess;
        hipError_t rc = set_dyn_lds(e, kern, bytes);
        if (rc == hipSuccess) rc = hipOccupancyMaxActiveBlocksPerMultiprocessor(blocks, kern, threads, bytes);
        if (rc == hipSuccess) cached.store(*blocks, std::memory_order_relaxed);
        return rc;
    }
};

template <int ENV, bool WIDE> hipError_t azg_persistent_search(azg_engine* e);
template <int ENV> hipError_t azg_lockstep_search(azg_engine* e);
template <int ENV> hipError_t azg_team_search(azg_engine* e);
hipError_t azg_team_wide_forms(azg_engine* e, int g_base, int G, bool dry, bool common, bool t32, bool t64);
hipError_t azg_dispatch_mlp_eval(azg_engine* e, const float* obs, int n, float* value, float* dist, float* raw);
```

### alphazero_gym_amd/csrc/records.h

```cpp
#pragma once
#include <hip/hip_runtime.h>
#include "../../include/azg_math.h"
#include "../../include/azgym.h"

#define FLAG_EXPANDED 1
#define FLAG_TERMINAL 2
#define TREES_PER_WG 16
#define MAX_STREAM_LAYERS 8

typedef float f32x4 __attribute__((ext_vector_type(4)));

struct __attribute__((aligned(16))) RecS {
    double Q;
    unsigned short edge_n;
    unsigned short node_n;
    unsigned char parent;
    unsigned char n_child : 5;
    unsigned char wnext : 1;
    unsigned char flags : 2;
    unsigned char first;
    unsigned char cbase;
};
#define POOL_UNITS(R) ((7 * ((R) - 1) + 8) / 9 + 1)
struct __attribute__((aligned(16))) RecM {
    double Q;
    unsigned long long edge_n : 11;
    unsigned long long node_n : 11;
    unsigned long long parent : 9;
    unsigned long long first : 9;
    unsigned long long cbase : 9;
    unsigned long long n_child : 5;
    unsigned long long flags : 2;
    unsigned long long wnext : 1;
};
static_assert(sizeof(RecM) == 16, "RecM must be 16 bytes");
#define TS_GLOBAL 0
#define TS_LDS8 1
#define TS_LDS9 2
struct __attribute__((aligned(8))) RecL {
    double Q;
    int edge_n;
    int node_n;
    short parent;
    unsigned short n_child;
    unsigned short first;
    unsigned char flags;
    unsigned char pad;
};
static_assert(sizeof(RecS) == 16, "RecS must be 16 bytes");
static_assert(sizeof(RecL) == 24, "RecL must be 24 bytes");

struct __attribute__((aligned(16))) Cold {
    double s[4];
    double r;
    float V;
    float mu;
    float sg;
    float pad;
};
static_assert(sizeof(Cold) == 64, "Cold must be 64 bytes");

struct KParams {
    int B, n_sims, R, Kp, A, nd, n_out, n_hidden, act, v1, tree_base, mode;
    double c_uct, gamma, epsilon, reward_scale;
    float c_uct_f, gamma_f, bound_f, ls_min, ls_max;
    unsigned long long seed;
    unsigned search_idx;
    int S;
    int tab_n;
    const double* roots;
    const int* carry;
    RecL* hot;
    Cold* cold;
    double* edge_W;
    float* action;
    float* prior;
    float* gmm;
    int ncomp;
    unsigned short* child;
    int* n_rec;
    const int* pw_need;
    const double* sqrt_tab;
    const f32x4* W0u;
    const f32x4* b0u;
    const float* W0;
    const float* W0b;
    int in8;
    const f32x4* b0;
    const f32x4* Wl[MAX_STREAM_LAYERS];
    const f32x4* bl[MAX_STREAM_LAYERS];
    const f32x4* Whead;
    const float* bhead;
    int layernorm;
    int Htrue[MAX_STREAM_LAYERS];
    const f32x4* lng[MAX_STREAM_LAYERS];
    const f32x4* lnb[MAX_STREAM_LAYERS];
    float* res_actions; int* res_counts; double* res_Q; double* res_vt; int* res_nch; int* res_child_n; double* res_child_state;
    float* res_root_V; float* res_root_dist;
    int res_Kmax, res_v_target;
    int tie_random;
    int env_id;
    int trace_cap;
    int lds_state;
    int pw0;
    int publish;
    unsigned long long* stamps;
    int net_T, net_wgs;
    size_t net_wstride;
};

struct LsLane { int my_depth, pid; double pr, pW; float eps_c; float pad; };
struct LsTree { int nrec; unsigned eps_draws; int leaf, need_eval, path_D, kbase; };

struct LockStep {
    float* obsT;
    f32x4* act[2];
    f32x4* parts;
    LsTree* tree;
    LsLane* lane;
};


#ifdef AZG_STAMPS
#ifdef AZG_STAMP_ONLY
#define STAMP_ON(s1, s2) ((s1) == (AZG_STAMP_ONLY) || (s2) == (AZG_STAMP_ONLY))
#else
#define STAMP_ON(s1, s2) 1
#endif
#define STAMP3(var, s1, s2, s3) [[maybe_unused]] unsigned long long var = 0; if constexpr (STAMP_ON(s1, s2) || STAMP_ON(s3, s3)) { var = __builtin_amdgcn_s_memtime(); __builtin_amdgcn_sched_barrier(0); }
#define STAMP2(var, s1, s2) STAMP3(var, s1, s2, -1)
#define STAMP(var) STAMP2(var, -2, -2)
#define STAMP_ADD(slot, t0, t1) do { if constexpr (STAMP_ON(slot, slot)) st_acc[slot] += (t1) - (t0); } while (0)
#define STAMP_PARAM , unsigned long long* st_acc
#define STAMP_ARG , st_acc
#ifdef AZG_STAMPS_A
#define STAMP_A(var, s1, s2) STAMP2(var, s1, s2)
#define STAMP_A_ADD(slot, t0, t1) do { if constexpr (STAMP_ON(slot, slot)) { if (st_acc) st_acc[slot] += (t1) - (t0); } } while (0)
#define STAMP_M(var, s1, s2) [[maybe_unused]] unsigned long long var = 0
#define STAMP_M_ADD(slot, t0, t1)
#else
#define STAMP_A(var, s1, s2)
#define STAMP_A_ADD(slot, t0, t1)
#define STAMP_M(var, s1, s2) STAMP2(var, s1, s2)
#define STAMP_M_ADD(slot, t0, t1) STAMP_ADD(slot, t0, t1)
#endif
#define STAMP_PARAM_OPT , unsigned long long* st_acc = nullptr
#else
#define STAMP_PARAM
#define STAMP_ARG
#define STAMP(var)
#define STAMP2(var, s1, s2)
#define STAMP3(var, s1, s2, s3)
#define STAMP_ADD(slot, t0, t1)
#define STAMP_A(var, s1, s2)
#define STAMP_A_ADD(slot, t0, t1)
#define STAMP_M(var, s1, s2)
#define STAMP_M_ADD(slot, t0, t1)
#define STAMP_PARAM_OPT
#endif
```

### alphazero_gym_amd/csrc/search_kernel.cuh

```cuda
#pragma once
#include "records.h"
#include "env.cuh"
#include "mlp.cuh"
#include "tree.cuh"
#include "tree_phases.cuh"
#include "results.cuh"
#ifndef AZG_DEFER
#define AZG_DEFER 1
#endif

struct LdsLayout {
    size_t act_off;
    size_t tree_off;
    size_t per_tree;
    size_t state_off;
    size_t total;
};
__host__ __device__ inline LdsLayout lds_layout(int tab_n, int n_sims, int HP, int NG, int nbuf, int R, bool cont, int tlds, int lds_state = 0, int NT = 16) {
    LdsLayout L;
    L.act_off = ((size_t)tab_n * 8 + (size_t)(n_sims + 2) * 2 + 15) / 16 * 16;
    L.tree_off = L.act_off + (size_t)nbuf * NG * HP * 64;
    L.per_tree = (size_t)R * 16 + (cont ? (size_t)POOL_UNITS(R) * (tlds == TS_LDS9 ? 8 : 4) : (size_t)R * 4);
    L.per_tree = (L.per_tree + 15) / 16 * 16;
    L.state_off = 0;
    if (lds_state && !cont && tlds != TS_GLOBAL) { L.state_off = L.per_tree; L.per_tree += (size_t)(n_sims + 1) * 32; }
    L.total = L.tree_off + (tlds != TS_GLOBAL ? L.per_tree * NT * NG : 0);
    return L;
}
__host__ __device__ constexpr int act_buffers(int NREG) { return NREG == 1 ? 1 : 2; }

template <int ENV, int HP, int NREG, int TLDS, bool GMM, int NW, int NG, int NT = 16, int SPEC = 0>
__global__ __launch_bounds__(64 * NW, NT < 16 ? 2 : 1) void search_kernel(KParams P) {
    constexpr bool CONT = EnvFamily<ENV>::CONT;
    static_assert(NT == 16 || (NG == 1 && NW == 4 && (NT == 8 || NT == 4)), "half-filled tiles: one group, four waves");
    constexpr int TPW = NT * NG;
    constexpr int NWALK = (NW == 8 && NG == 1) ? 4 : NW;
    constexpr int TPV = TPW / NWALK;
    typedef typename TreeStore<TLDS>::Rec Rec;
    constexpr int NCH = head_chunks<HP>();
    constexpr int PSTR = GMM ? 64 : 16;
    __shared__ f32x4 s_parts[NG * NCH * PSTR];
    constexpr bool IN8 = EnvFamily<ENV>::IN8;
    __shared__ float s_obsT[(IN8 ? 8 : 4) * TPW];
    __shared__ float s_bhead[16];
    __shared__ float s_ln[NREG == 0 ? 2 * 64 : 1];
    __shared__ int s_done;
    constexpr bool DEFER = AZG_DEFER && NW == 8 && NG == 1 && ENV == AZG_ENV_PENDULUM_V1 && TLDS != TS_GLOBAL && NREG > 0 && !GMM && HP <= 256;
    __shared__ int s_l0;
    extern __shared__ double s_dyn[];

    const int tid = threadIdx.x;
    const int wave = tid >> 6, lane = tid & 63;
    const int wnet = (int)blockIdx.x / P.net_wgs;
    const int wj0 = ((int)blockIdx.x - wnet * P.net_wgs) * TPW;
    const int tree0 = wnet * P.net_T + wj0;
    const int n_live = (P.net_T - wj0) < TPW ? (P.net_T - wj0) : TPW;
    const size_t wofs = (size_t)wnet * P.net_wstride;
    constexpr bool LEAN = (NW == 8);
    const LdsLayout L = lds_layout(P.tab_n, P.n_sims, HP, NG, act_buffers(NREG), P.R, CONT, TLDS, P.lds_state, NT);
    double* s_sqrt = s_dyn;
    unsigned short* s_pw = (unsigned short*)(s_dyn + P.tab_n);
    f32x4* s_actA = (f32x4*)((char*)s_dyn + L.act_off);
    f32x4* s_actB = act_buffers(NREG) == 2 ? s_actA + NG * (HP / 16 * 64) : s_actA;
    for (int i = tid; i < P.tab_n; i += 64 * NW) s_sqrt[i] = P.sqrt_tab[i];
    if (CONT) for (int i = tid; i < P.n_sims + 2; i += 64 * NW) s_pw[i] = (unsigned short)(P.pw_need[i] < 65535 ? P.pw_need[i] : 65535);
    if (tid < 16) s_bhead[tid] = P.bhead[wofs + tid];
    if (tid == 0) { s_done = 0; s_l0 = 0; }

    typedef WRegs<HP, NREG, NW, DEFER> WR;
    WR wr;
    constexpr int NTW = HP / (16 * NW);
    if constexpr (DEFER) {
        if (wave >= NW / 2) {
#pragma unroll
            for (int i = 0; i < 2 * NTW; ++i) {
                wr.w0[i] = P.W0[wofs + ((wave - NW / 2) * 2 * NTW + i) * 64 + lane];
                wr.b0[i] = net_ptr(P.b0, wofs)[((wave - NW / 2) * 2 * NTW + i) * 64 + lane];
            }
        }
    } else if constexpr (HP <= 256) {
#pragma unroll
        for (int i = 0; i < NTW; ++i) {
            wr.w0[i] = P.W0[wofs + (wave * NTW + i) * 64 + lane];
            if constexpr (IN8) { if (P.in8) wr.w0b[i] = P.W0b[wofs + (wave * NTW + i) * 64 + lane]; }
            wr.b0[i] = net_ptr(P.b0, wofs)[(wave * NTW + i) * 64 + lane];
        }
    }
    if (NREG > 0) {
        constexpr int S4 = HP / 16;
#pragma unroll
        for (int l = 0; l < NREG; ++l) {
#pragma unroll
            for (int i = 0; i < NTW; ++i) {
                wr.b[l][i] = net_ptr(P.bl[l], wofs)[(wave * NTW + i) * 64 + lane];
#pragma unroll
                for (int s4 = 0; s4 < S4; ++s4) wr.w[l][i][s4] = net_ptr(P.Wl[l], wofs)[((wave * NTW + i) * S4 + s4) * 64 + lane];
            }
        }
#pragma unroll
        for (int i = 0; i < NTW; ++i) wr.wh[i] = net_ptr(P.Whead, wofs)[(wave * NTW + i) * 64 + lane];
    }

    struct Ctx {
        int sub, tl, tree; bool has_tree, live; unsigned gtree; size_t tb;
        Cold* cold; double* edge_W; float* action; TreeStore<TLDS> ts; const f32x4* my_parts;
    };
    auto make_ctx = [&](int t) {
        Ctx c;
        const int w = t >> 6, ln = t & 63;
        c.sub = ln & 15;
        c.has_tree = w < NWALK && (ln >> 4) < TPV;
        c.tl = c.has_tree ? w * TPV + (ln >> 4) : 0;
        c.tree = tree0 + c.tl;
        c.live = c.has_tree && c.tl < n_live;
        c.gtree = (unsigned)(P.tree_base + c.tree);
        c.tb = (size_t)(c.live ? c.tree : 0) * P.R;
        c.cold = P.cold + c.tb;
        c.edge_W = P.edge_W + c.tb;
        c.action = P.action + c.tb;
        if constexpr (TLDS != TS_GLOBAL) {
            char* base = (char*)s_dyn + L.tree_off + L.per_tree * c.tl;
            c.ts.hot = (Rec*)base;
            c.ts.pool = (typename TreeStore<TLDS>::PoolId*)(base + (size_t)P.R * 16);
            c.ts.prior = (float*)(base + (size_t)P.R * 16);
            c.ts.state = L.state_off ? (double*)(base + L.state_off) : nullptr;
        } else {
            c.ts.hot = (Rec*)(P.hot + c.tb);
            c.ts.child = P.child + c.tb * P.Kp;
            c.ts.prior = P.prior + c.tb;
        }
        c.my_parts = s_parts + (c.tl / NT) * NCH * PSTR;
        return c;
    };
    Ctx cx = make_ctx(tid);

#ifdef AZG_STAMPS
    unsigned long long st_acc[16] = {0, 0, 0, 0, 0, 0, 0, 0, 0, 0, 0, 0, 0, 0, 0, 0};
#endif
    TreeState st = {};
    st.need_eval = false;
    BDeferred bdef = {};
    if (cx.has_tree) tree_init_root<ENV, TLDS, TPW, IN8>(P, st, cx.ts, cx.cold, cx.edge_W, cx.action, cx.tree, cx.live, cx.sub, cx.tl, cx.gtree, s_obsT);
    __syncthreads();

    constexpr bool MULTI = !CONT;
    static_assert(!(LEAN && MULTI), "discrete 8-wave shapes: extend the LEAN packing first");
    int my_sim = -1;
    for (int sim = -1; sim < P.n_sims; ++sim) {
        STAMP2(t_a, 0, -1);
        __syncthreads();
        if constexpr (MULTI) { if (*(volatile int*)&s_done >= n_live) break; }
        STAMP2(t_b, 0, 1);
        if constexpr (DEFER) {
            STAMP2(t_b2a, 12, -1);
            if (cx.live) tree_phase_b2<ENV, TLDS, SPEC>(P, st, cx.ts, cx.cold, cx.edge_W, cx.action, bdef, cx.sub, cx.gtree, s_pw);
            bdef.pending = false;
            STAMP2(t_b2b, 12, -1);
#ifdef AZG_STAMP_ONLY
            STAMP_ADD(12, t_b2a, t_b2b);
#endif
        }
        unsigned pk0 = 0, pk1 = 0, pk2 = 0, pk3 = 0;
        int tid_o = tid;
        if constexpr (LEAN) {
            pk0 = (unsigned)st.nrec | ((unsigned)st.leaf << 16);
            pk1 = (unsigned)st.path_D | ((unsigned)st.kbase << 16);
            pk2 = (unsigned)(st.my_depth + 1) | ((unsigned)st.pid << 16);
            pk3 = (unsigned)st.ptop | ((unsigned)st.need_eval << 16) | ((unsigned)st.resume << 20);
            asm volatile("" : "+v"(pk0), "+v"(pk1), "+v"(pk2), "+v"(pk3));
        }
#ifdef AZG_STAMPS
        mlp_forward<HP, NREG, NW, NG, PSTR, WR, NT, IN8, DEFER>(P, wr, s_obsT, s_actA, s_actB, s_parts, s_ln, wave, lane, st_acc, &s_l0, sim + 2, wofs);
#else
        mlp_forward<HP, NREG, NW, NG, PSTR, WR, NT, IN8, DEFER>(P, wr, s_obsT, s_actA, s_actB, s_parts, s_ln, wave, lane, &s_l0, sim + 2, wofs);
#endif
        STAMP2(t_c, 1, 2);
        if constexpr (LEAN) {
            asm volatile("" : "+v"(pk0), "+v"(pk1), "+v"(pk2), "+v"(pk3), "+v"(tid_o));
            st.nrec = (int)(pk0 & 0xffffu); st.leaf = (int)(pk0 >> 16);
            st.path_D = (int)(pk1 & 0xffffu); st.kbase = (int)(pk1 >> 16);
            st.my_depth = (int)(pk2 & 0xffffu) - 1; st.pid = (int)(pk2 >> 16);
            st.ptop = (int)(pk3 & 0xffffu); st.need_eval = ((pk3 >> 16) & 1u) != 0; st.resume = (int)(pk3 >> 20);
            cx = make_ctx(tid_o);
            st.pr = 0.0; st.pW = 0.0;
            if (cx.live && (MULTI ? my_sim : sim) >= 0 && st.my_depth >= 1) {
                st.pr = CONT ? cx.cold[st.pid].r : discrete_env_reward(Spec<SPEC, ENV>::env(P));
                st.pW = cx.edge_W[st.pid];
            }
        }
        if constexpr (!MULTI) {
            if (cx.live) tree_phase_a<ENV, TLDS, GMM, NCH, PSTR, !CONT, SPEC>(P, st, cx.ts, cx.cold, cx.edge_W, cx.action, cx.tb, sim, cx.sub, cx.tl % NT, cx.gtree, cx.my_parts, s_bhead, s_sqrt STAMP_ARG, s_pw);
            if (sim == P.n_sims - 1) break;
            if constexpr (DEFER) { if (sim < 0 && cx.live) eps_prepare(P, st, cx.gtree, cx.sub); }
            tree_fence();
            STAMP2(t_d, 2, 3);
            st.need_eval = false;
            if (cx.live) tree_phase_b<ENV, TLDS, GMM, TPW, unsigned short, !LEAN, !CONT, SPEC, IN8, DEFER>(P, st, cx.ts, cx.cold, cx.edge_W, cx.action, cx.tb, cx.sub, cx.tl, cx.gtree, s_sqrt, s_pw, s_obsT STAMP_ARG, &bdef);
            tree_fence();
            STAMP2(t_e, 3, -1);
            STAMP_ADD(2, t_c, t_d);
            STAMP_ADD(3, t_d, t_e);
        } else {
            bool run = cx.live && my_sim < P.n_sims;
            int k = 0;
            while (run) {
                STAMP2(t_c2, 2, -1);
                tree_phase_a<ENV, TLDS, GMM, NCH, PSTR, !CONT, SPEC>(P, st, cx.ts, cx.cold, cx.edge_W, cx.action, cx.tb, my_sim, cx.sub, cx.tl % NT, cx.gtree, cx.my_parts, s_bhead, s_sqrt STAMP_ARG, s_pw);
                tree_fence();
                STAMP2(t_d, 2, 3);
                st.need_eval = false;
                if (my_sim == P.n_sims - 1) {
                    my_sim = P.n_sims;
                    if (cx.sub == 0) atomicAdd(&s_done, 1);
                    run = false;
                } else {
                    my_sim += 1;
                    tree_phase_b<ENV, TLDS, GMM, TPW, unsigned short, !LEAN, !CONT, SPEC, IN8>(P, st, cx.ts, cx.cold, cx.edge_W, cx.action, cx.tb, cx.sub, cx.tl, cx.gtree, s_sqrt, s_pw, s_obsT STAMP_ARG);
                    tree_fence();
                    k += 1;
                    if (st.need_eval || k >= P.trace_cap) run = false;
                }
                STAMP2(t_e, 3, -1);
                STAMP_ADD(2, t_c2, t_d);
                STAMP_ADD(3, t_d, t_e);
            }
        }
        STAMP_ADD(0, t_a, t_b);
        STAMP_ADD(1, t_b, t_c);
    }
    const int nrec = st.nrec;
    const int sub = cx.sub, tree = cx.tree;
    const bool live = cx.live;
    const size_t tb = cx.tb;
    const TreeStore<TLDS>& ts = cx.ts;
#ifdef AZG_STAMPS
    if (lane == 0) for (int i = 0; i < 16; ++i) P.stamps[((size_t)blockIdx.x * NW + wave) * 16 + i] = st_acc[i];
#endif
    if (live) results_for_tree<CONT, TLDS>(P, ts, cx.cold, cx.action, tb, tree, sub);
    if (live) {
        if (sub == 0) P.n_rec[tree] = nrec;
        if constexpr (TLDS != TS_GLOBAL) {
            if (P.publish) {
                RecL* gh = P.hot + tb;
                for (int j = sub; j < nrec; j += 16) {
                    Rec h = ts.hot[j];
                    RecL o;
                    o.Q = h.Q; o.edge_n = h.edge_n; o.node_n = h.node_n; o.parent = (short)h.parent; o.n_child = h.n_child;
                    o.first = CONT ? 0 : h.first; o.flags = h.flags; o.pad = 0;
                    gh[j] = o;
                    if (CONT) {
                        for (int i = 0; i < (int)h.n_child; ++i) P.child[(tb + j) * P.Kp + i] = (unsigned short)ts.child_at(j, h, i, P.Kp);
                    } else {
                        P.prior[tb + j] = ts.prior[j];
                    }
                }
            }
        }
    }
}
```

### alphazero_gym_amd/csrc/tree.cuh

```cuda
#pragma once
#include "records.h"

__device__ __forceinline__ void tree_fence() { __builtin_amdgcn_fence(__ATOMIC_ACQ_REL, "wavefront"); }

__device__ __forceinline__ double tree_div(double n, double d) {
    double r = __builtin_amdgcn_rcp(d);
    double e = __builtin_fma(-d, r, 1.0);
    r = __builtin_fma(r, e, r);
    e = __builtin_fma(-d, r, 1.0);
    r = __builtin_fma(r, e, r);
    double q = n * r;
    double rem = __builtin_fma(-d, q, n);
    return __builtin_fma(rem, r, q);
}


template <int CTRL>
__device__ __forceinline__ int dpp_i32(int v) { return __builtin_amdgcn_update_dpp(0, v, CTRL, 0xf, 0xf, false); }
template <int CTRL>
__device__ __forceinline__ double dpp_f64(double v) {
    unsigned long long u = azg_d2u(v);
    unsigned lo = (unsigned)dpp_i32<CTRL>((int)(unsigned)u), hi = (unsigned)dpp_i32<CTRL>((int)(unsigned)(u >> 32));
    return azg_u2d(((unsigned long long)hi << 32) | lo);
}
template <int CTRL>
__device__ __forceinline__ float dpp_f32(float v) { return __builtin_bit_cast(float, dpp_i32<CTRL>(__builtin_bit_cast(int, v))); }
#define DPP_QUAD_BCAST1 0x55
#define DPP_QUAD_XOR1 0xB1
#define DPP_QUAD_XOR2 0x4E
#define DPP_ROW_ROR4 0x124
#define DPP_ROW_ROR8 0x128
#define DPP_ROW_ROR15 0x12F

__device__ __forceinline__ double rowmax16(double u, bool valid) {
    double m = valid ? u : -__builtin_huge_val();
    double o;
    o = dpp_f64<DPP_QUAD_XOR1>(m); m = o > m ? o : m;
    o = dpp_f64<DPP_QUAD_XOR2>(m); m = o > m ? o : m;
    o = dpp_f64<DPP_ROW_ROR4>(m); m = o > m ? o : m;
    o = dpp_f64<DPP_ROW_ROR8>(m); m = o > m ? o : m;
    return m;
}
__device__ __forceinline__ int rowmin16(int c) {
    int t;
    t = dpp_i32<DPP_QUAD_XOR1>(c); c = t < c ? t : c;
    t = dpp_i32<DPP_QUAD_XOR2>(c); c = t < c ? t : c;
    t = dpp_i32<DPP_ROW_ROR4>(c); c = t < c ? t : c;
    t = dpp_i32<DPP_ROW_ROR8>(c); c = t < c ? t : c;
    return c;
}
__device__ __forceinline__ int argmax16(double u, bool valid, int sub) {
    double m = rowmax16(u, valid);
    return rowmin16((valid && u == m) ? sub : 99);
}
__device__ __forceinline__ int rowmax16_i32(int v) {
    int o;
    o = dpp_i32<DPP_QUAD_XOR1>(v); v = o > v ? o : v;
    o = dpp_i32<DPP_QUAD_XOR2>(v); v = o > v ? o : v;
    o = dpp_i32<DPP_ROW_ROR4>(v); v = o > v ? o : v;
    o = dpp_i32<DPP_ROW_ROR8>(v); v = o > v ? o : v;
    return v;
}
__device__ __forceinline__ unsigned rowmax16_u32(unsigned v) {
    unsigned o;
    o = (unsigned)dpp_i32<DPP_QUAD_XOR1>((int)v); v = o > v ? o : v;
    o = (unsigned)dpp_i32<DPP_QUAD_XOR2>((int)v); v = o > v ? o : v;
    o = (unsigned)dpp_i32<DPP_ROW_ROR4>((int)v); v = o > v ? o : v;
    o = (unsigned)dpp_i32<DPP_ROW_ROR8>((int)v); v = o > v ? o : v;
    return v;
}
__device__ __forceinline__ int argmax16_payload(double u, bool valid, int sub, int payload) {
    const long long bits = (long long)azg_d2u(u);
    const long long key = bits ^ ((bits >> 63) & 0x7fffffffffffffffLL);
    const int hi = valid ? (int)(key >> 32) : (int)0x80000000;
    const unsigned lo = (unsigned)key;
    const int mh = rowmax16_i32(hi);
    const bool top = valid && hi == mh;
    const unsigned ml = rowmax16_u32(top ? lo : 0u);
    return rowmin16((top && lo == ml) ? ((sub << 16) | payload) : 0x7fffffff) & 0xffff;
}

#define DPP_QUAD_BCAST0 0x00
__device__ __forceinline__ int argmax2_payload(double u, int sub, int payload) {
    const double o = dpp_f64<DPP_QUAD_XOR1>(u);
    const int po = dpp_i32<DPP_QUAD_XOR1>(payload);
    int w = (sub == 0) ? (u >= o ? payload : po) : 0;
    w = dpp_i32<DPP_QUAD_BCAST0>(w);
    int t = dpp_i32<DPP_ROW_ROR4>(w); w = t > w ? t : w;
    t = dpp_i32<DPP_ROW_ROR8>(w); w = t > w ? t : w;
    return w;
}

template <int TLDS> struct TreeStore;
template <typename RecT, typename IdT> struct TreeStoreLds {
    typedef RecT Rec;
    typedef IdT PoolId;
    Rec* hot; IdT* pool; float* prior;
    double* state;
    __device__ __forceinline__ int child_at(int, const Rec& hp, int i, int) const {
        return hp.n_child == 1 ? (int)hp.first : (int)pool[4 * (int)hp.cbase + i];
    }
    __device__ __forceinline__ void child_append(int p, const Rec& hp, int K, int id, int& ptop, bool writer, int, bool wnext = false) const {
        const int cb = hp.cbase;
        if (K == 0) {
            if (writer) hot[p].first = (decltype(hp.first))id;
        } else if (K == 1 || K == 4 || K == 8) {
            const int nb = ptop;
            ptop += K == 1 ? 1 : K / 2;
            if (writer) {
                if (K == 1) pool[4 * nb] = (IdT)hp.first;
                else for (int w = 0; w < K; ++w) pool[4 * nb + w] = pool[4 * cb + w];
                pool[4 * nb + K] = (IdT)id;
                hot[p].cbase = (decltype(hp.cbase))nb;
            }
        } else {
            if (writer) pool[4 * cb + K] = (IdT)id;
        }
        if (writer) { hot[p].n_child = (decltype(hp.n_child))(K + 1); hot[p].wnext = wnext ? 1 : 0; }
    }
};
template <> struct TreeStore<TS_LDS8> : TreeStoreLds<RecS, unsigned char> {};
template <> struct TreeStore<TS_LDS9> : TreeStoreLds<RecM, unsigned short> {};
template <> struct TreeStore<TS_GLOBAL> {
    typedef RecL Rec;
    Rec* hot; unsigned short* child; float* prior;
    static constexpr double* state = nullptr;
    __device__ __forceinline__ int child_at(int p, const Rec&, int i, int Kp) const { return (int)child[p * Kp + i]; }
    __device__ __forceinline__ void child_append(int p, const Rec&, int K, int id, int&, bool writer, int Kp, bool wnext = false) const {
        if (writer) {
            child[p * Kp + K] = (unsigned short)id;
            hot[p].n_child = (unsigned short)(K + 1);
            hot[p].pad = wnext ? 1 : 0;
        }
    }
};

__device__ __forceinline__ bool get_wnext(const RecS& h) { return h.wnext != 0; }
__device__ __forceinline__ bool get_wnext(const RecM& h) { return h.wnext != 0; }
__device__ __forceinline__ bool get_wnext(const RecL& h) { return (h.pad & 1) != 0; }
__device__ __forceinline__ void set_wnext(RecS& h, bool w) { h.wnext = w ? 1 : 0; }
__device__ __forceinline__ void set_wnext(RecM& h, bool w) { h.wnext = w ? 1 : 0; }
__device__ __forceinline__ void set_wnext(RecL& h, bool w) { h.pad = w ? 1 : 0; }
template <typename PW>
__device__ __forceinline__ int pw_at(const PW* s_pw, int n, int cap) { return (int)s_pw[n < cap ? n : cap]; }

template <typename Rec>
__device__ __forceinline__ Rec make_edge(double Q, int parent) {
    Rec h;
    h.Q = Q; h.edge_n = 0; h.node_n = 0; h.parent = (decltype(h.parent))parent; h.n_child = 0; h.flags = 0; h.first = 0;
    set_wnext(h, false);
    return h;
}
__device__ __forceinline__ void clear_pad(RecS& h) { h.cbase = 0; }
__device__ __forceinline__ void clear_pad(RecM& h) { h.cbase = 0; }
__device__ __forceinline__ void clear_pad(RecL& h) { h.pad = 0; }

template <bool CONT, int TLDS, typename F, typename PW = int>
__device__ __forceinline__ void backup_from(const TreeStore<TLDS>& ts, const Cold* cold, double* edge_W, int j, float V, int sub,
                                            float gamma_f, double gamma, bool firstlvl, bool at_leaf, double Rv, F&& on_node,
                                            const PW* s_pw = nullptr, int pw_cap = 0) {
    typedef typename TreeStore<TLDS>::Rec Rec;
    while (true) {
        int mine = 0, cnt = 0, jj = j;
        bool hit_root = false;
#pragma unroll 1
        for (int d = 0; d < 16; ++d) {
            if (sub == d) mine = jj;
            cnt = d + 1;
            if (jj == 0) { hit_root = true; break; }
            jj = ts.hot[jj].parent;
        }
        Rec mrec = ts.hot[mine];
        const bool is_edge = (sub < cnt) && (mine != 0);
        double r = 0.0, W = 0.0;
        if (is_edge) { r = cold[mine].r; W = edge_W[mine]; }
        double myR = 0.0;
        const int nedge = hit_root ? cnt - 1 : cnt;
#pragma unroll 1
        for (int d = 0; d < nedge; ++d) {
            double rd = __shfl(r, d, 16);
            double gR;
            if (firstlvl) {
                gR = CONT ? (double)(gamma_f * V) : gamma * (double)V;
                firstlvl = false;
            } else {
                gR = gamma * Rv;
            }
            Rv = rd + gR;
            if (sub == d) myR = Rv;
        }
        if (sub < cnt) {
            if (is_edge) {
                int en = (int)mrec.edge_n + 1;
                double Wn = W + myR;
                mrec.Q = tree_div(Wn, (double)en);
                mrec.edge_n = (decltype(mrec.edge_n))en;
                edge_W[mine] = Wn;
            }
            if (!(at_leaf && sub == 0)) {
                mrec.node_n = (decltype(mrec.node_n))(mrec.node_n + 1);
                if constexpr (CONT) set_wnext(mrec, pw_at(s_pw, (int)mrec.node_n, pw_cap) - (int)mrec.n_child > 0);
            }
            ts.hot[mine] = mrec;
        }
        if (!TLDS) tree_fence();
        for (int d = 0; d < cnt; ++d) {
            const int pn = __shfl(mine, d, 16);
            if (!(at_leaf && d == 0)) on_node(pn);
        }
        if (hit_root) break;
        j = jj;
        at_leaf = false;
    }
}

template <bool CONT, int TLDS, typename F, typename PW = int>
__device__ __forceinline__ void backup_path(const TreeStore<TLDS>& ts, const Cold* cold, double* edge_W, float V, int sub, float gamma_f,
                                            double gamma, int D, int my_depth, int pid, double pr, double& pW, F&& on_node,
                                            typename TreeStore<TLDS>::Rec& rec, double& chainR, bool same_chain = false,
                                            double r_uniform = 0.0, double r_first = 0.0, const PW* s_pw = nullptr, int pw_cap = 0) {
    typedef typename TreeStore<TLDS>::Rec Rec;
    const int n0 = D < 16 ? D : 16;
    double Rv = 0.0, myR = 0.0;
    if (same_chain) {
        myR = chainR;
    } else if constexpr (!CONT) {
        double R = 0.0;
        if (gamma == 1.0) {
            const float av = __builtin_fabsf(V);
            if (av == 0.0f || (av >= 0x1p-25f && av < 0x1p30f)) {
                const int dl = (D - sub) & 15;
                if (dl < n0) myR = (r_first + (double)dl * r_uniform) + (double)V;
                R = n0 > 0 ? (r_first + (double)(n0 - 1) * r_uniform) + (double)V : (double)V;
            } else {
                R = (double)V;
#pragma unroll 2
                for (int d = 0; d < n0; ++d) {
                    R = (d == 0 ? r_first : r_uniform) + R;
                    if (sub == ((D - d) & 15)) myR = R;
                }
            }
        } else {
#pragma unroll 2
            for (int d = 0; d < n0; ++d) {
                const double gR = d == 0 ? gamma * (double)V : gamma * R;
                R = (d == 0 ? r_first : r_uniform) + gR;
                if (sub == ((D - d) & 15)) myR = R;
            }
        }
        Rv = R;
        chainR = myR;
    } else {
#pragma unroll 1
        for (int d = 0; d < n0; ++d) {
            const int src = (D - d) & 15;
            const double nb = dpp_f64<DPP_ROW_ROR15>(myR);
            const double gR = d == 0 ? (CONT ? (double)(gamma_f * V) : gamma * (double)V) : gamma * nb;
            if (sub == src) myR = pr + gR;
        }
        chainR = myR;
    }
    if (CONT && D >= 16) Rv = __shfl(myR, (D - 15) & 15, 16);
    const bool valid = my_depth >= 0 && my_depth > D - 16;
    int par = 0;
    rec = make_edge<Rec>(0.0, 0);
    clear_pad(rec);
    if (valid) {
        rec = ts.hot[pid];
        int need = 0;
        if constexpr (CONT) { if (my_depth < D) need = pw_at(s_pw, (int)rec.node_n + 1, pw_cap); }
        par = rec.parent;
        if (my_depth >= 1) {
            int en = (int)rec.edge_n + 1;
            double Wn = pW + myR;
            rec.Q = tree_div(Wn, (double)en);
            rec.edge_n = (decltype(rec.edge_n))en;
            edge_W[pid] = Wn;
            pW = Wn;
        }
        if (my_depth < D) {
            rec.node_n = (decltype(rec.node_n))(rec.node_n + 1);
            if constexpr (CONT) set_wnext(rec, need - (int)rec.n_child > 0);
        }
        ts.hot[pid] = rec;
    }
    if (D >= 16) {
        int j = __shfl(par, (D - 15) & 15, 16);
        backup_from<CONT, TLDS>(ts, cold, edge_W, j, V, sub, gamma_f, gamma, false, false, Rv, on_node, s_pw, pw_cap);
    }
}
```

### alphazero_gym_amd/csrc/tree_phases.cuh

```cuda
#pragma once
#ifndef EARLY_COLD
#define EARLY_COLD 1
#endif
#include "records.h"
#include "env.cuh"
#include "mlp.cuh"
#include "tree.cuh"

struct TreeState {
    int nrec;
    unsigned eps_draws;
    int leaf;
    bool need_eval;
    int path_D;
    int my_depth, pid;
    double pr, pW;
    int kbase;
    float eps_c;
    float eps_next;
    int ptop;
    int resume;
    double chainR;
    bool repeat;
};

template <int SPEC, int ENV = AZG_ENV_CARTPOLE> struct Spec {
    static __device__ __forceinline__ bool eps0(const KParams& P) { return SPEC ? true : P.epsilon == 0.0; }
    static __device__ __forceinline__ bool tie_random(const KParams& P) { return SPEC ? false : P.tie_random != 0; }
    static __device__ __forceinline__ bool plain(const KParams& P) { return SPEC ? true : (P.epsilon == 0.0 && !P.tie_random); }
    static __device__ __forceinline__ int A(const KParams& P) { return ENV == AZG_ENV_ACROBOT ? 3 : (SPEC ? 2 : P.A); }
    static __device__ __forceinline__ int env(const KParams& P) {
        return ENV == AZG_ENV_ACROBOT ? (int)AZG_ENV_ACROBOT : (SPEC ? (int)AZG_ENV_CARTPOLE : P.env_id);
    }
    static __device__ __forceinline__ int v1(const KParams& P) { return SPEC ? 1 : P.v1; }
    static __device__ __forceinline__ bool in_table(const KParams& P, int n) { return SPEC ? true : n < P.tab_n; }
};

template <bool CONT> __device__ __forceinline__ int rec_best(const RecS& h) { return CONT ? (int)h.first : (int)h.first + (int)h.cbase; }
template <bool CONT> __device__ __forceinline__ int rec_best(const RecM& h) { return CONT ? (int)h.first : (int)h.first + (int)h.cbase; }
template <bool CONT> __device__ __forceinline__ int rec_best(const RecL& h) { return CONT ? (int)h.first : (int)h.first + (int)h.pad; }
template <bool CONT> __device__ __forceinline__ void set_best(RecS* r, const RecS& h, int c) {
    if (CONT) r->first = (unsigned char)c; else r->cbase = (unsigned char)(c - (int)h.first);
}
template <bool CONT> __device__ __forceinline__ void set_best(RecM* r, const RecM& h, int c) {
    if (CONT) r->first = (unsigned)c; else r->cbase = (unsigned)(c - (int)h.first);
}
template <bool CONT> __device__ __forceinline__ void set_best(RecL* r, const RecL& h, int c) {
    if (CONT) r->first = (unsigned short)c; else r->pad = (unsigned char)(c - (int)h.first);
}

template <int ENV, int TLDS, typename Rec, int SPEC = 0>
__device__ __forceinline__ int select_child(const KParams& P, const TreeStore<TLDS>& ts, int p, const Rec& hp, int sub, const double* s_sqrt,
                                            int pick, unsigned gtree = 0u) {
    constexpr bool CONT = EnvFamily<ENV>::CONT;
    const int K = hp.n_child;
    double sq;
    if (CONT || Spec<SPEC, ENV>::in_table(P, (int)hp.node_n)) sq = s_sqrt[hp.node_n];
    else sq = __builtin_sqrt((double)((int)hp.node_n + 1));
    int win_c = 0;
    if (TLDS || K <= 16) {
        const bool valid = sub < K;
        const int si = valid ? sub : 0;
        int c = CONT ? ts.child_at(p, hp, si, P.Kp) : (int)hp.first + si;
        if (!valid) c = 0;
        Rec h = ts.hot[c];
        double ratio = tree_div(sq, (double)((int)h.edge_n + 1));
        double U;
        if (CONT) {
            U = h.Q + P.c_uct * ratio;
        } else {
            float pc = ts.prior[c] * P.c_uct_f;
            U = h.Q + (double)pc * ratio;
        }
        if (!SPEC && pick >= 0) win_c = __shfl(c, pick, 16);
        else if (!CONT && K == 2) win_c = argmax2_payload(U, sub, c);
        else win_c = argmax16_payload(U, valid, sub, c);
        if (Spec<SPEC, ENV>::tie_random(P) && pick < 0) {
            const double m = rowmax16(U, valid);
            const unsigned row = (unsigned)(__ballot(valid && U == m) >> (threadIdx.x & 48)) & 0xffffu;
            const int cnt = __popc(row);
            if (cnt > 1) {
                const azg_u32x4 b = azg_draw(P.seed, gtree, P.search_idx, ((unsigned)hp.node_n << 16) ^ (unsigned)p, AZG_STREAM_TIE);
                int kth = (int)(b.v[0] % (unsigned)cnt);
                unsigned r2 = row;
                while (kth-- > 0) r2 &= r2 - 1;
                win_c = __shfl(c, __builtin_ctz(r2), 16);
            }
        }
    } else {
        double win_u = 0.0;
        bool have = false;
        for (int base = 0; base < K; base += 16) {
            const int i = base + sub;
            const bool valid = i < K;
            int c = 0;
            double U = 0.0;
            if (valid) {
                c = CONT ? ts.child_at(p, hp, i, P.Kp) : (int)hp.first + i;
                Rec h = ts.hot[c];
                double ratio = tree_div(sq, (double)((int)h.edge_n + 1));
                if (CONT) {
                    U = h.Q + P.c_uct * ratio;
                } else {
                    float pc = ts.prior[c] * P.c_uct_f;
                    U = h.Q + (double)pc * ratio;
                }
            }
            int w;
            if (pick >= 0) w = (pick >= base && pick < base + 16) ? pick - base : -1;
            else w = argmax16(U, valid, sub);
            if (w >= 0) {
                int wc = __shfl(c, w, 16);
                double wu = __shfl(U, w, 16);
                if (pick >= 0 || !have || wu > win_u) { win_c = wc; win_u = wu; have = true; }
            }
        }
    }
    return win_c;
}

template <int ENV, int TLDS, int SPEC = 0>
__device__ __forceinline__ void refresh_best(const KParams& P, const TreeStore<TLDS>& ts, int p, int sub, const double* s_sqrt) {
    constexpr bool CONT = EnvFamily<ENV>::CONT;
    typedef typename TreeStore<TLDS>::Rec Rec;
    const Rec hp = ts.hot[p];
    const int b = select_child<ENV, TLDS, Rec, SPEC>(P, ts, p, hp, sub, s_sqrt, -1);
    if (sub == 0) set_best<CONT>(&ts.hot[p], hp, b);
}

template <int ENV, int TLDS, int SPEC = 0>
__device__ __forceinline__ int refresh_best_own_slot(const KParams& P, const TreeStore<TLDS>& ts, int pid, bool mine, const double* s_sqrt,
                                                     const typename TreeStore<TLDS>::Rec& hp) {
    typedef typename TreeStore<TLDS>::Rec Rec;
    const int p = mine ? pid : 0;
    double sq;
    if (Spec<SPEC, ENV>::in_table(P, (int)hp.node_n)) sq = s_sqrt[hp.node_n];
    else sq = __builtin_sqrt((double)((int)hp.node_n + 1));
    const int c0 = (int)hp.first;
    const Rec h0 = ts.hot[c0], h1 = ts.hot[c0 + 1];
    const float pc0 = ts.prior[c0] * P.c_uct_f, pc1 = ts.prior[c0 + 1] * P.c_uct_f;
    const double U0 = h0.Q + (double)pc0 * tree_div(sq, (double)((int)h0.edge_n + 1));
    const double U1 = h1.Q + (double)pc1 * tree_div(sq, (double)((int)h1.edge_n + 1));
    const int win = c0 + (U0 >= U1 ? 0 : 1);
    if (mine) set_best<false>(&ts.hot[p], hp, win);
    return win;
}

template <int ENV, int TLDS, int TPW = 16, bool OBS8 = false>
__device__ __forceinline__ void tree_init_root(const KParams& P, TreeState& st, const TreeStore<TLDS>& ts, Cold* cold, double* edge_W,
                                               float* action, int tree, bool live, int sub, int tl, unsigned gtree, float* obsT) {
    constexpr bool CONT = EnvFamily<ENV>::CONT;
    constexpr int S = CONT ? 2 : 4;
    typedef typename TreeStore<TLDS>::Rec Rec;
    st.nrec = 1; st.eps_draws = 0; st.leaf = 0; st.need_eval = live;
    st.path_D = 0; st.my_depth = -1; st.pid = 0; st.pr = 0.0; st.pW = 0.0;
    st.kbase = 1; st.eps_c = 0.0f; st.eps_next = 0.0f; st.ptop = 0; st.resume = 0; st.chainR = 0.0; st.repeat = false;
    if (CONT && live) st.eps_c = azg_normal(P.seed, gtree, P.search_idx, (unsigned)(st.kbase + sub));
        double rs[S], sn;
#pragma unroll
        for (int k = 0; k < S; ++k) rs[k] = (live && k < P.S) ? P.roots[(size_t)tree * P.S + k] : 0.0;
        float obs[OBS8 ? 8 : 4];
        if constexpr (OBS8) { sn = 0.0; azg_acrobot_obs(rs, obs); obs[6] = 0.0f; obs[7] = 0.0f; }
        else env_obs<ENV == AZG_ENV_ACROBOT ? AZG_ENV_CARTPOLE : ENV>(rs, obs, &sn);
        if (live && sub == 0) {
            Rec h = make_edge<Rec>(0.0, 0);
            h.node_n = (decltype(h.node_n))P.carry[tree];
            h.flags = FLAG_EXPANDED;
            clear_pad(h);
            if (CONT) set_wnext(h, pw_at(P.pw_need, (int)P.carry[tree], P.n_sims + 1) > 0);
            ts.hot[0] = h;
            Cold c;
#pragma unroll
            for (int k = 0; k < 4; ++k) c.s[k] = k < S ? rs[k] : 0.0;
            if (CONT) c.s[2] = sn;
            c.r = 0.0; c.V = 0.0f; c.mu = 0.0f; c.sg = 0.0f; c.pad = 0.0f;
            cold[0] = c;
            edge_W[0] = 0.0;
            if (CONT) action[0] = 0.0f;
            if constexpr (!CONT && TLDS != TS_GLOBAL) {
                if (ts.state) {
#pragma unroll
                    for (int k = 0; k < 4; ++k) ts.state[k] = rs[k];
                }
            }
        }
        if constexpr (!OBS8) {
            if (sub < 4) obsT[sub * TPW + tl] = live ? obs[sub] : 0.0f;
        } else if (sub < 8) {
            float v = sub == 0 ? obs[0] : (sub == 1 ? obs[1] : (sub == 2 ? obs[2] : obs[3]));
            if (sub >= 4) v = sub == 4 ? obs[4] : (sub == 5 ? obs[5] : (sub == 6 ? obs[6] : obs[7]));
            obsT[sub * TPW + tl] = live ? v : 0.0f;
        }
}

template <int ENV, int TLDS, bool GMM, int NCH, int PSTR = 64, bool RESUME = false, int SPEC = 0, typename PW = int>
__device__ __forceinline__ void tree_phase_a(const KParams& P, TreeState& st, const TreeStore<TLDS>& ts, Cold* cold, double* edge_W,
                                             float* action, size_t tb, int sim, int sub, int tl, unsigned gtree, const f32x4* parts,
                                             const float* bhead, const double* s_sqrt STAMP_PARAM_OPT, const PW* s_pw = nullptr) {
    constexpr bool CONT = EnvFamily<ENV>::CONT;
    typedef typename TreeStore<TLDS>::Rec Rec;
    float V = 0.0f;
    STAMP_A(ta0, 4, -1);
    if (st.need_eval) {
        f32x4 out4 = {0.0f, 0.0f, 0.0f, 0.0f};
        if constexpr (!CONT) { out4 = head_output4<NCH, PSTR>(parts, bhead, tl); V = out4.x; }
        else V = head_output<NCH, PSTR>(parts, bhead, tl, 0);
        if (CONT) {
            float mu, sg;
            float gd[15];
            if constexpr (GMM) {
                gmm_params<NCH, PSTR>(parts, bhead, tl, P.ncomp, P.ls_min, P.ls_max, gd);
                mu = gd[0]; sg = gd[GMM_MAXC];
                float* g = P.gmm + (tb + st.leaf) * 3 * GMM_MAXC;
                if (sub == 0) {
#pragma unroll
                    for (int i = 0; i < 3 * GMM_MAXC; ++i) g[i] = gd[i];
                }
            } else {
                mu = head_output<NCH, PSTR>(parts, bhead, tl, 1);
                float ls = head_output<NCH, PSTR>(parts, bhead, tl, 2);
                ls = ls < P.ls_min ? P.ls_min : (ls > P.ls_max ? P.ls_max : ls);
                sg = azg_expf(ls);
            }
            if (sub == 0) { cold[st.leaf].V = V; cold[st.leaf].mu = mu; cold[st.leaf].sg = sg; }
            if (sim < 0) {
                int k = st.nrec++;
                if constexpr (GMM) gmm_pick(gd, P.ncomp, P.seed, gtree, P.search_idx, (unsigned)k, &mu, &sg);
                float eps = __shfl(st.eps_c, k - st.kbase, 16);
                float a = P.bound_f * azg_tanhf(mu + sg * eps);
                if (sub == 0) {
                    Rec h = make_edge<Rec>((double)V, 0);
                    clear_pad(h);
                    ts.hot[k] = h;
                    edge_W[k] = 0.0;
                    action[k] = a;
                }
                ts.child_append(0, make_edge<Rec>(0.0, 0), 0, k, st.ptop, sub == 0, P.Kp,
                                pw_at(P.pw_need, (int)ts.hot[0].node_n, P.n_sims + 1) - 1 > 0);
            }
        } else {
            const int A = Spec<SPEC, ENV>::A(P);
            float my_logit = sub == 0 ? out4.y : (sub == 1 ? out4.z : out4.w);
            if (A > 3 && sub >= 3 && sub < A) my_logit = head_output<NCH, PSTR>(parts, bhead, tl, 1 + sub);
            float mx = out4.y;
            if (A == 2) {
                mx = out4.z > mx ? out4.z : mx;
            } else {
                for (int a = 1; a < A; ++a) { const float v = __shfl(my_logit, a, 16); mx = v > mx ? v : mx; }
            }
            const float e_mine = azg_expf(my_logit - mx);
            float sum;
            if (A == 2) {
                sum = dpp_f32<DPP_QUAD_BCAST0>(e_mine) + dpp_f32<DPP_QUAD_BCAST1>(e_mine);
            } else {
                sum = 0.0f;
                for (int a = 0; a < A; ++a) sum = sum + __shfl(e_mine, a, 16);
            }
            int k0 = st.nrec;
            st.nrec += A;
            if (sub < A) {
                float prior_a = e_mine / sum;
                Rec h = make_edge<Rec>((double)V, st.leaf);
                clear_pad(h);
                ts.hot[k0 + sub] = h;
                ts.prior[k0 + sub] = prior_a;
                edge_W[k0 + sub] = 0.0;
            }
            if (sub == 0) {
                cold[st.leaf].V = V;
                ts.hot[st.leaf].n_child = (decltype(ts.hot[st.leaf].n_child))A;
                ts.hot[st.leaf].first = (decltype(ts.hot[st.leaf].first))k0;
            }
            if (Spec<SPEC, ENV>::plain(P)) {
                if (A == 2) {
                    const int nn = (int)ts.hot[st.leaf].node_n;
                    double sq;
                    if (Spec<SPEC, ENV>::in_table(P, nn)) sq = s_sqrt[nn];
                    else sq = __builtin_sqrt((double)(nn + 1));
                    float prior_s = 0.0f;
                    if (sub < A) prior_s = e_mine / sum;
                    const float pc = prior_s * P.c_uct_f;
                    const double U = (double)V + (double)pc * sq;
                    const double o = dpp_f64<DPP_QUAD_XOR1>(U);
                    if (sub == 0) set_best<false>(&ts.hot[st.leaf], make_edge<Rec>(0.0, 0), U >= o ? 0 : 1);
                } else {
                    if (!TLDS) tree_fence();
                    refresh_best<ENV, TLDS, SPEC>(P, ts, st.leaf, sub, s_sqrt);
                }
            }
        }
    }
    STAMP_A(ta1, 4, 5);
    STAMP_A_ADD(4, ta0, ta1);
    if (sim >= 0) {
        if (!TLDS) tree_fence();
        const bool keep = !CONT && Spec<SPEC, ENV>::plain(P);
        Rec myrec;
        backup_path<CONT, TLDS>(ts, cold, edge_W, V, sub, P.gamma_f, P.gamma, st.path_D, st.my_depth, st.pid, st.pr, st.pW,
                                [&](int pn) { if (keep) refresh_best<ENV, TLDS, SPEC>(P, ts, pn, sub, s_sqrt); }, myrec, st.chainR,
                                RESUME && !CONT && st.repeat,
                                CONT ? 0.0 : discrete_env_reward(Spec<SPEC, ENV>::env(P)),
                                CONT ? 0.0 : (st.need_eval ? discrete_env_reward(Spec<SPEC, ENV>::env(P)) : discrete_env_terminal_reward(Spec<SPEC, ENV>::env(P))),
                                s_pw, P.n_sims + 1);
        STAMP_A(ta2, 5, 6);
        STAMP_A_ADD(5, ta1, ta2);
        if constexpr (!CONT) {
            if (keep) {
                const int D = st.path_D, lo = D > 15 ? D - 15 : 0;
                if (!TLDS) tree_fence();
                if (Spec<SPEC, ENV>::A(P) == 2) {
                    const bool mine = st.my_depth >= lo && st.my_depth < D;
                    const int win = refresh_best_own_slot<ENV, TLDS, SPEC>(P, ts, st.pid, mine, s_sqrt, myrec);
                    if constexpr (RESUME) {
                        const int next_pid = dpp_i32<DPP_ROW_ROR15>(st.pid);
                        const unsigned long long votes = __ballot(mine && win != next_pid);
                        const unsigned row = (unsigned)(votes >> (threadIdx.x & 48)) & 0xffffu;
                        st.resume = D < 16 ? (row ? __builtin_ctz(row) : D) : 0;
                    }
                } else {
                    for (int d = D - 1; d >= lo; --d) refresh_best<ENV, TLDS, SPEC>(P, ts, __shfl(st.pid, d & 15, 16), sub, s_sqrt);
                }
            }
        }
        STAMP_A(ta3, 6, -1);
        STAMP_A_ADD(6, ta2, ta3);
    }
}

__device__ __forceinline__ void eps_prepare(const KParams& P, TreeState& st, unsigned gtree, int sub) {
    if (st.nrec >= st.kbase + 16) {
        st.kbase = st.nrec;
        st.eps_c = azg_normal(P.seed, gtree, P.search_idx, (unsigned)(st.kbase + sub));
    }
    st.eps_next = __shfl(st.eps_c, st.nrec - st.kbase, 16);
}

struct BDeferred {
    bool pending, widen;
    int p, chosen;
    float cact;
};

template <int ENV, int TLDS, int SPEC, bool FETCH = false, typename PW = int>
__device__ __forceinline__ void tree_phase_b2(const KParams& P, TreeState& st, const TreeStore<TLDS>& ts, Cold* cold, double* edge_W, float* action,
                                              const BDeferred& d, int sub, unsigned gtree, const PW* s_pw) {
    typedef typename TreeStore<TLDS>::Rec Rec;
    static_assert(ENV == AZG_ENV_PENDULUM_V1, "deferred expansion: the Pendulum family");
    if (!d.pending) return;
    const double ps0 = cold[d.p].s[0], ps1 = cold[d.p].s[1];
    if (d.widen) {
        const float V = cold[d.p].V;
        const Rec hp = ts.hot[d.p];
        if (sub == 0) {
            Rec h = make_edge<Rec>((double)V, d.p);
            h.flags = FLAG_EXPANDED;
            clear_pad(h);
            set_wnext(h, P.pw0 > 0);
            ts.hot[d.chosen] = h;
            edge_W[d.chosen] = 0.0;
            action[d.chosen] = d.cact;
        }
        ts.child_append(d.p, hp, (int)hp.n_child, d.chosen, st.ptop, sub == 0, P.Kp,
                        pw_at(s_pw, (int)hp.node_n, P.n_sims + 1) - ((int)hp.n_child + 1) > 0);
    } else if (sub == 0) {
        Rec h = ts.hot[d.chosen];
        h.flags = FLAG_EXPANDED;
        set_wnext(h, P.pw0 > 0);
        ts.hot[d.chosen] = h;
    }
    const double sp[2] = {ps0, ps1};
    const double r = pendulum_reward(sp, d.cact) / P.reward_scale;
    if constexpr (FETCH) { if (sub == (st.path_D & 15)) st.pr = r; }
    if (sub == 0) {
        float zero = 0.0f;
        asm volatile("" : "+v"(zero));
        Cold* c = cold + d.chosen;
        c->s[3] = 0.0; c->r = r; c->V = zero; c->mu = zero; c->sg = zero; c->pad = zero;
    }
    eps_prepare(P, st, gtree, sub);
}

template <int ENV, int TLDS, bool GMM, int TPW = 16, typename PW = int, bool FETCH = true, bool RESUME = false, int SPEC = 0, bool OBS8 = false, bool DEFER = false>
__device__ __forceinline__ void tree_phase_b(const KParams& P, TreeState& st, const TreeStore<TLDS>& ts, Cold* cold, double* edge_W,
                                             float* action, size_t tb, int sub, int tl, unsigned gtree, const double* s_sqrt,
                                             const PW* s_pw, float* obsT STAMP_PARAM, BDeferred* def = nullptr) {
    static_assert(!DEFER || (ENV == AZG_ENV_PENDULUM_V1 && !GMM), "deferred expansion: Pendulum family, squashed-Normal head");
    constexpr bool CONT = EnvFamily<ENV>::CONT;
    constexpr int S = CONT ? 2 : 4;
    typedef typename TreeStore<TLDS>::Rec Rec;
    st.need_eval = false;
    if (CONT && !DEFER && st.nrec >= st.kbase + 16) {
        st.kbase = st.nrec;
        st.eps_c = azg_normal(P.seed, gtree, P.search_idx, (unsigned)(st.kbase + sub));
    }
    int p = 0;
    bool resumed = false;
    st.repeat = false;
    if constexpr (RESUME && !CONT) {
        if (Spec<SPEC, ENV>::plain(P) && Spec<SPEC, ENV>::A(P) == 2 && st.resume > 0) {
            resumed = true;
            p = __shfl(st.pid, st.resume, 16);
            if (st.my_depth > st.resume) st.my_depth = -1;
            st.path_D = st.resume;
        }
    }
    const double r_step = CONT ? 0.0 : discrete_env_reward(Spec<SPEC, ENV>::env(P));
    const bool keep_slot = !CONT && FETCH && resumed && st.my_depth >= 1;
    Rec hp = ts.hot[p];
    Cold cp;
    bool from_cold = true;
    if constexpr (!CONT && TLDS != TS_GLOBAL) from_cold = (ts.state == nullptr);
    if (from_cold) cp = cold[p];
    else { cp.s[0] = cp.s[1] = cp.s[2] = cp.s[3] = 0.0; }
    if (!resumed) { st.path_D = 0; st.my_depth = sub == 0 ? 0 : -1; st.pid = 0; }
    if (!keep_slot) { st.pr = 0.0; st.pW = 0.0; }
    int chosen = 0;
    bool widen = false, hit_terminal = false;
    if constexpr (RESUME && !CONT) {
        hit_terminal = resumed && (hp.flags & FLAG_TERMINAL);
        st.repeat = FETCH && hit_terminal;
    }
    STAMP2(tb0, 13, -1);
    while (!hit_terminal) {
        STAMP3(tl0, 7, 8, 11);
        const int K = hp.n_child;
        if (CONT) {
            widen = get_wnext(hp);
            if (widen) break;
        }
        if (CONT || !Spec<SPEC, ENV>::plain(P)) {
            int pick = -1;
            if (!Spec<SPEC, ENV>::eps0(P)) {
                azg_u32x4 b = azg_draw(P.seed, gtree, P.search_idx, st.eps_draws++, AZG_STREAM_EPS);
                if ((double)azg_u01(b.v[0]) < P.epsilon) pick = (int)(b.v[1] % (unsigned)K);
            }
            chosen = select_child<ENV, TLDS, Rec, SPEC>(P, ts, p, hp, sub, s_sqrt, pick, gtree);
        } else {
            chosen = rec_best<CONT>(hp);
        }
        STAMP2(tl1, 7, -1);
        STAMP_ADD(7, tl0, tl1);
        STAMP2(tl2, 8, 9);
        Cold cn;
        if constexpr (CONT && EARLY_COLD) cn = cold[chosen];
        Rec hc = ts.hot[chosen];
        if (!(hc.flags & FLAG_EXPANDED)) break;
        STAMP2(tl3, 9, 10);
        st.path_D += 1;
        p = chosen;
        hp = hc;
        if (sub == (st.path_D & 15)) {
            st.my_depth = st.path_D; st.pid = chosen;
            if (CONT && FETCH) { st.pr = EARLY_COLD ? cn.r : cold[chosen].r; st.pW = edge_W[chosen]; }
            if (!CONT && FETCH) { st.pr = r_step; st.pW = edge_W[chosen]; }
        }
        if constexpr (EnvFamily<ENV>::TERM) {
            if (hc.flags & FLAG_TERMINAL) { hit_terminal = true; break; }
        }
        if (CONT) { if constexpr (EARLY_COLD) cp = cn; else cp = cold[p]; }
        else if (from_cold) { cp.s[0] = cold[p].s[0]; cp.s[1] = cold[p].s[1]; cp.s[2] = cold[p].s[2]; cp.s[3] = cold[p].s[3]; }
        STAMP2(tl4, 10, 11);
        STAMP_ADD(8, tl0, tl2);
        STAMP_ADD(9, tl2, tl3);
        STAMP_ADD(10, tl3, tl4);
        STAMP_ADD(11, tl0, tl4);
#if defined(AZG_STAMPS) && !defined(AZG_STAMP_ONLY)
        st_acc[12] += 1;
#endif
    }
    STAMP2(tb1, 13, 14);
    STAMP_ADD(13, tb0, tb1);
    if (hit_terminal) {
        st.leaf = p;
    } else {
        float cact = 0.0f;
        if (widen) {
            const int K = hp.n_child;
            chosen = st.nrec++;
            float eps = DEFER ? st.eps_next : __shfl(st.eps_c, chosen - st.kbase, 16);
            float wmu = cp.mu, wsg = cp.sg;
            if constexpr (GMM) {
                float gd[15];
                const float* g = P.gmm + (tb + p) * 3 * GMM_MAXC;
#pragma unroll
                for (int i = 0; i < 3 * GMM_MAXC; ++i) gd[i] = g[i];
                gmm_pick(gd, P.ncomp, P.seed, gtree, P.search_idx, (unsigned)chosen, &wmu, &wsg);
            }
            cact = P.bound_f * azg_tanhf(wmu + wsg * eps);
            if constexpr (!DEFER) {
                if (sub == 0) {
                    Rec h = make_edge<Rec>((double)cp.V, p);
                    clear_pad(h);
                    ts.hot[chosen] = h;
                    edge_W[chosen] = 0.0;
                    action[chosen] = cact;
                }
                ts.child_append(p, hp, K, chosen, st.ptop, sub == 0, P.Kp, pw_at(s_pw, (int)hp.node_n, P.n_sims + 1) - (K + 1) > 0);
            }
        }
        STAMP2(tw1, 14, 15);
        STAMP_ADD(14, tb1, tw1);
        st.path_D += 1;
        double ns[S], r, sn;
        int done;
        if (CONT) {
            if (!widen) cact = action[chosen];
            if constexpr (DEFER) {
                pendulum_dynamics(Spec<SPEC, ENV>::v1(P), cp.s, cp.s[2], cact, ns);
                r = 0.0; done = 0;
            } else {
                if constexpr (ENV == AZG_ENV_MOUNTAINCAR_CONT) mountaincar_cont_step(cp.s, cact, ns, &r, &done);
                else pendulum_step(Spec<SPEC, ENV>::v1(P), cp.s, cp.s[2], cact, ns, &r, &done);
                r = r / P.reward_scale;
            }
        } else {
            if constexpr (TLDS != TS_GLOBAL) {
                if (ts.state) {
                    const int slot = Spec<SPEC, ENV>::A(P) == 2 ? ((int)hp.first - 1) >> 1 : ((int)hp.first - 1) / P.A;
                    const double* sp = ts.state + 4 * slot;
                    cp.s[0] = sp[0]; cp.s[1] = sp[1]; cp.s[2] = sp[2]; cp.s[3] = sp[3];
                }
            }
            family_env_step<ENV>(Spec<SPEC, ENV>::env(P), cp.s, chosen - (int)hp.first, ns, &r, &done);
        }
        float obs[OBS8 ? 8 : 4];
        if constexpr (OBS8) { sn = 0.0; azg_acrobot_obs(ns, obs); obs[6] = 0.0f; obs[7] = 0.0f; }
        else env_obs<ENV == AZG_ENV_ACROBOT ? AZG_ENV_CARTPOLE : ENV>(ns, obs, &sn);
        STAMP2(tw2, 15, -1);
        STAMP_ADD(15, tw1, tw2);
        if constexpr (DEFER) {
            def->pending = true; def->widen = widen; def->p = p; def->chosen = chosen; def->cact = cact;
            if (sub == 0) { cold[chosen].s[0] = ns[0]; cold[chosen].s[1] = ns[1]; cold[chosen].s[2] = sn; }
        } else if (sub == 0) {
            Cold c;
#pragma unroll
            for (int k = 0; k < 4; ++k) c.s[k] = k < S ? ns[k] : 0.0;
            if (CONT) c.s[2] = sn;
            float zero = 0.0f;
            asm volatile("" : "+v"(zero));
            c.r = r; c.V = zero; c.mu = zero; c.sg = zero; c.pad = zero;
            cold[chosen] = c;
            if constexpr (CONT) {
                Rec hn = ts.hot[chosen];
                hn.flags = (unsigned char)(FLAG_EXPANDED | (done ? FLAG_TERMINAL : 0));
                set_wnext(hn, P.pw0 > 0);
                ts.hot[chosen] = hn;
            } else {
                ts.hot[chosen].flags = (unsigned char)(FLAG_EXPANDED | (done ? FLAG_TERMINAL : 0));
            }
            if constexpr (!CONT && TLDS != TS_GLOBAL) {
                if (ts.state && !done) {
                    double* sp = ts.state + 4 * (Spec<SPEC, ENV>::A(P) == 2 ? (st.nrec - 1) >> 1 : (st.nrec - 1) / P.A);
#pragma unroll
                    for (int k = 0; k < 4; ++k) sp[k] = ns[k];
                }
            }
        }
        if (sub == (st.path_D & 15)) { st.my_depth = st.path_D; st.pid = chosen; st.pr = r; st.pW = 0.0; }
        st.leaf = chosen;
        st.need_eval = !done;
        if constexpr (!OBS8) {
            if (sub < 4) obsT[sub * TPW + tl] = done ? 0.0f : obs[sub];
        } else if (sub < 8) {
            float v = sub == 0 ? obs[0] : (sub == 1 ? obs[1] : (sub == 2 ? obs[2] : obs[3]));
            if (sub >= 4) v = sub == 4 ? obs[4] : (sub == 5 ? obs[5] : (sub == 6 ? obs[6] : obs[7]));
            obsT[sub * TPW + tl] = done ? 0.0f : v;
        }
    }
}
```

Baseline: 546.4 million sims/s.

## Add LDS warm ring for recent node states and move edge W into LDS

For the deferred-expansion Pendulum kernels, this adds a per-tree LDS region holding edge W values and a small ring of recently created nodes' states and policy heads (Warm records). Selection reads node state from this ring, falling back to the global cold record only for nodes that have left the ring. Backup reads and writes edge W in LDS, and the values are copied to global memory at the end. The aim is to cut global memory latency on the selection and backup paths, at the cost of extra LDS per tree; the ring size is reduced when needed so the kernel can keep the same occupancy.

Measured after the change: 534.5 million sims/s. 0.978x the previous value.

```diff
diff --git a/alphazero_gym_amd/csrc/azg_engine.hip b/alphazero_gym_amd/csrc/azg_engine.hip
--- a/alphazero_gym_amd/csrc/azg_engine.hip
+++ b/alphazero_gym_amd/csrc/azg_engine.hip
@@ -214,6 +214,7 @@
     { const char* v = getenv("AZG_TEAM_TT"); e->opt.team_tt = v ? atoi(v) : 0; }
     { const char* v = getenv("AZG_TEAM_SPIN_LIMIT"); e->opt.team_spin_limit = v ? atol(v) : (1L << 23); }
     e->opt.no_lds_state = getenv("AZG_NO_LDS_STATE") != nullptr;
+    { const char* v = getenv("AZG_WARM_SLOTS"); const int t = v ? atoi(v) : -1; e->opt.warm_slots = t >= 0 ? t : -1; }
     e->d_team_cnt = nullptr; e->team_cnt_bytes = 0; e->team_pending = 0; e->team_fallbacks = 0; e->team_search_idx = 0;
     e->lds_warned = 0; e->last_search_idx = 0; e->ms_kept = 0.0f; e->ms_kept_valid = 0;
     e->carry_max = 0;
diff --git a/alphazero_gym_amd/csrc/dispatch.cuh b/alphazero_gym_amd/csrc/dispatch.cuh
--- a/alphazero_gym_amd/csrc/dispatch.cuh
+++ b/alphazero_gym_amd/csrc/dispatch.cuh
@@ -21,7 +21,13 @@
     const size_t room = 160 * 1024 - (size_t)static_lds;
     const bool costs_a_neighbour = n_wg > e->n_cus && 2 * (without.total + static_lds) <= 160 * 1024 && 2 * (with_state.total + static_lds) > 160 * 1024;
     e->P.lds_state = (!CONT && TLDS != TS_GLOBAL && with_state.total <= room && !costs_a_neighbour && !e->opt.no_lds_state) ? 1 : 0;
-    const size_t lds = e->P.lds_state ? with_state.total : without.total;
+    size_t lds = e->P.lds_state ? with_state.total : without.total;
+    e->P.warm_slots = -1;
+    if constexpr (search_kernel_defer(ENV, HP, NREG, TLDS, GMM, NW, NG)) {
+        const WarmPlan w = warm_plan(e->tab_n, e->cfg.n_sims, HP, NG, act_buffers(NREG), e->R, TLDS, NT, static_lds, n_wg, e->n_cus, e->opt.warm_slots);
+        e->P.warm_slots = w.slots;
+        lds = w.lds;
+    }
     if (lds > room) return hipErrorInvalidConfiguration;
     rc = attrs.set_dyn_lds(e, (const void*)kern, lds);
     if (rc != hipSuccess) return rc;
diff --git a/alphazero_gym_amd/csrc/engine_host.h b/alphazero_gym_amd/csrc/engine_host.h
--- a/alphazero_gym_amd/csrc/engine_host.h
+++ b/alphazero_gym_amd/csrc/engine_host.h
@@ -21,6 +21,7 @@
     int team_wide;
     int team_tt;
     long team_spin_limit;
+    int warm_slots;
     int no_lds_state;
 };
 #define AZG_MAX_DEVICES 64
diff --git a/alphazero_gym_amd/csrc/records.h b/alphazero_gym_amd/csrc/records.h
--- a/alphazero_gym_amd/csrc/records.h
+++ b/alphazero_gym_amd/csrc/records.h
@@ -59,6 +59,12 @@
     float pad;
 };
 static_assert(sizeof(Cold) == 64, "Cold must be 64 bytes");
+struct __attribute__((aligned(16))) Warm {
+    double s[3];
+    float mu, sg;
+};
+static_assert(sizeof(Warm) == 32, "Warm must be 32 bytes");
+#define AZG_WARM_SLOTS_MAX 64
 
 struct KParams {
     int B, n_sims, R, Kp, A, nd, n_out, n_hidden, act, v1, tree_base, mode;
@@ -102,6 +108,7 @@
     int env_id;
     int trace_cap;
     int lds_state;
+    int warm_slots;
     int pw0;
     int publish;
     unsigned long long* stamps;
diff --git a/alphazero_gym_amd/csrc/search_kernel.cuh b/alphazero_gym_amd/csrc/search_kernel.cuh
--- a/alphazero_gym_amd/csrc/search_kernel.cuh
+++ b/alphazero_gym_amd/csrc/search_kernel.cuh
@@ -14,9 +14,12 @@
     size_t tree_off;
     size_t per_tree;
     size_t state_off;
+    size_t w_off;
+    size_t warm_off;
     size_t total;
 };
-__host__ __device__ inline LdsLayout lds_layout(int tab_n, int n_sims, int HP, int NG, int nbuf, int R, bool cont, int tlds, int lds_state = 0, int NT = 16) {
+__host__ __device__ constexpr int warm_ring_slots(int M) { return (M > 1 ? M : 1) + 1; }
+__host__ __device__ inline LdsLayout lds_layout(int tab_n, int n_sims, int HP, int NG, int nbuf, int R, bool cont, int tlds, int lds_state = 0, int NT = 16, int warm_slots = -1) {
     LdsLayout L;
     L.act_off = ((size_t)tab_n * 8 + (size_t)(n_sims + 2) * 2 + 15) / 16 * 16;
     L.tree_off = L.act_off + (size_t)nbuf * NG * HP * 64;
@@ -24,10 +27,32 @@
     L.per_tree = (L.per_tree + 15) / 16 * 16;
     L.state_off = 0;
     if (lds_state && !cont && tlds != TS_GLOBAL) { L.state_off = L.per_tree; L.per_tree += (size_t)(n_sims + 1) * 32; }
+    L.w_off = L.warm_off = 0;
+    if (warm_slots >= 0 && cont && tlds != TS_GLOBAL) {
+        L.w_off = L.per_tree;
+        L.warm_off = L.w_off + ((size_t)R * 8 + 15) / 16 * 16;
+        L.per_tree = L.warm_off + (size_t)warm_ring_slots(warm_slots) * sizeof(Warm);
+    }
     L.total = L.tree_off + (tlds != TS_GLOBAL ? L.per_tree * NT * NG : 0);
     return L;
 }
+struct WarmPlan { int slots; size_t lds; };
+inline WarmPlan warm_plan(int tab_n, int n_sims, int HP, int NG, int nbuf, int R, int tlds, int NT, int static_lds, long n_wg, int n_cus, int want) {
+    auto total = [&](int m) { return lds_layout(tab_n, n_sims, HP, NG, nbuf, R, true, tlds, 0, NT, m).total; };
+    const size_t cu = 160 * 1024;
+    int M = AZG_WARM_SLOTS_MAX;
+    if (want >= 0 && want < M) M = want;
+    while (M & (M - 1)) M &= M - 1;
+    const bool two_fit = n_wg > n_cus && 2 * (total(0) + static_lds) <= cu;
+    while (M > 0 && (total(M) + static_lds > cu || (two_fit && 2 * (total(M) + static_lds) > cu))) M >>= 1;
+    return {M, total(M)};
+}
+
 __host__ __device__ constexpr int act_buffers(int NREG) { return NREG == 1 ? 1 : 2; }
+
+__host__ __device__ constexpr bool search_kernel_defer(int ENV, int HP, int NREG, int TLDS, bool GMM, int NW, int NG) {
+    return AZG_DEFER && NW == 8 && NG == 1 && ENV == AZG_ENV_PENDULUM_V1 && TLDS != TS_GLOBAL && NREG > 0 && !GMM && HP <= 256;
+}
 
 template <int ENV, int HP, int NREG, int TLDS, bool GMM, int NW, int NG, int NT = 16, int SPEC = 0>
 __global__ __launch_bounds__(64 * NW, NT < 16 ? 2 : 1) void search_kernel(KParams P) {
@@ -45,7 +70,8 @@
     __shared__ float s_bhead[16];
     __shared__ float s_ln[NREG == 0 ? 2 * 64 : 1];
     __shared__ int s_done;
-    constexpr bool DEFER = AZG_DEFER && NW == 8 && NG == 1 && ENV == AZG_ENV_PENDULUM_V1 && TLDS != TS_GLOBAL && NREG > 0 && !GMM && HP <= 256;
+    constexpr bool DEFER = search_kernel_defer(ENV, HP, NREG, TLDS, GMM, NW, NG);
+    constexpr bool WARM = DEFER;
     __shared__ int s_l0;
     extern __shared__ double s_dyn[];
 
@@ -57,7 +83,7 @@
     const int n_live = (P.net_T - wj0) < TPW ? (P.net_T - wj0) : TPW;
     const size_t wofs = (size_t)wnet * P.net_wstride;
     constexpr bool LEAN = (NW == 8);
-    const LdsLayout L = lds_layout(P.tab_n, P.n_sims, HP, NG, act_buffers(NREG), P.R, CONT, TLDS, P.lds_state, NT);
+    const LdsLayout L = lds_layout(P.tab_n, P.n_sims, HP, NG, act_buffers(NREG), P.R, CONT, TLDS, P.lds_state, NT, WARM ? P.warm_slots : -1);
     double* s_sqrt = s_dyn;
     unsigned short* s_pw = (unsigned short*)(s_dyn + P.tab_n);
     f32x4* s_actA = (f32x4*)((char*)s_dyn + L.act_off);
@@ -124,6 +150,7 @@
             c.ts.pool = (typename TreeStore<TLDS>::PoolId*)(base + (size_t)P.R * 16);
             c.ts.prior = (float*)(base + (size_t)P.R * 16);
             c.ts.state = L.state_off ? (double*)(base + L.state_off) : nullptr;
+            if constexpr (WARM) { c.ts.lw = (double*)(base + L.w_off); c.ts.warm = (Warm*)(base + L.warm_off); c.ts.wm = P.warm_slots; }
         } else {
             c.ts.hot = (Rec*)(P.hot + c.tb);
             c.ts.child = P.child + c.tb * P.Kp;
@@ -140,7 +167,7 @@
     TreeState st = {};
     st.need_eval = false;
     BDeferred bdef = {};
-    if (cx.has_tree) tree_init_root<ENV, TLDS, TPW, IN8>(P, st, cx.ts, cx.cold, cx.edge_W, cx.action, cx.tree, cx.live, cx.sub, cx.tl, cx.gtree, s_obsT);
+    if (cx.has_tree) tree_init_root<ENV, TLDS, TPW, IN8, WARM>(P, st, cx.ts, cx.cold, cx.edge_W, cx.action, cx.tree, cx.live, cx.sub, cx.tl, cx.gtree, s_obsT);
     __syncthreads();
 
     constexpr bool MULTI = !CONT;
@@ -153,7 +180,7 @@
         STAMP2(t_b, 0, 1);
         if constexpr (DEFER) {
             STAMP2(t_b2a, 12, -1);
-            if (cx.live) tree_phase_b2<ENV, TLDS, SPEC>(P, st, cx.ts, cx.cold, cx.edge_W, cx.action, bdef, cx.sub, cx.gtree, s_pw);
+            if (cx.live) tree_phase_b2<ENV, TLDS, SPEC, false, unsigned short, WARM>(P, st, cx.ts, cx.cold, cx.edge_W, cx.action, bdef, cx.sub, cx.gtree, s_pw);
             bdef.pending = false;
             STAMP2(t_b2b, 12, -1);
 #ifdef AZG_STAMP_ONLY
@@ -185,17 +212,18 @@
             st.pr = 0.0; st.pW = 0.0;
             if (cx.live && (MULTI ? my_sim : sim) >= 0 && st.my_depth >= 1) {
                 st.pr = CONT ? cx.cold[st.pid].r : discrete_env_reward(Spec<SPEC, ENV>::env(P));
-                st.pW = cx.edge_W[st.pid];
+                if constexpr (WARM) st.pW = cx.ts.lw[st.pid];
+                else st.pW = cx.edge_W[st.pid];
             }
         }
         if constexpr (!MULTI) {
-            if (cx.live) tree_phase_a<ENV, TLDS, GMM, NCH, PSTR, !CONT, SPEC>(P, st, cx.ts, cx.cold, cx.edge_W, cx.action, cx.tb, sim, cx.sub, cx.tl % NT, cx.gtree, cx.my_parts, s_bhead, s_sqrt STAMP_ARG, s_pw);
+            if (cx.live) tree_phase_a<ENV, TLDS, GMM, NCH, PSTR, !CONT, SPEC, unsigned short, WARM>(P, st, cx.ts, cx.cold, cx.edge_W, cx.action, cx.tb, sim, cx.sub, cx.tl % NT, cx.gtree, cx.my_parts, s_bhead, s_sqrt STAMP_ARG, s_pw);
             if (sim == P.n_sims - 1) break;
             if constexpr (DEFER) { if (sim < 0 && cx.live) eps_prepare(P, st, cx.gtree, cx.sub); }
             tree_fence();
             STAMP2(t_d, 2, 3);
             st.need_eval = false;
-            if (cx.live) tree_phase_b<ENV, TLDS, GMM, TPW, unsigned short, !LEAN, !CONT, SPEC, IN8, DEFER>(P, st, cx.ts, cx.cold, cx.edge_W, cx.action, cx.tb, cx.sub, cx.tl, cx.gtree, s_sqrt, s_pw, s_obsT STAMP_ARG, &bdef);
+            if (cx.live) tree_phase_b<ENV, TLDS, GMM, TPW, unsigned short, !LEAN, !CONT, SPEC, IN8, DEFER, WARM>(P, st, cx.ts, cx.cold, cx.edge_W, cx.action, cx.tb, cx.sub, cx.tl, cx.gtree, s_sqrt, s_pw, s_obsT STAMP_ARG, &bdef);
             tree_fence();
             STAMP2(t_e, 3, -1);
             STAMP_ADD(2, t_c, t_d);
@@ -239,6 +267,9 @@
     if (live) results_for_tree<CONT, TLDS>(P, ts, cx.cold, cx.action, tb, tree, sub);
     if (live) {
         if (sub == 0) P.n_rec[tree] = nrec;
+        if constexpr (WARM) {
+            for (int j = sub; j < nrec; j += 16) cx.edge_W[j] = ts.lw[j];
+        }
         if constexpr (TLDS != TS_GLOBAL) {
             if (P.publish) {
                 RecL* gh = P.hot + tb;
diff --git a/alphazero_gym_amd/csrc/tree.cuh b/alphazero_gym_amd/csrc/tree.cuh
--- a/alphazero_gym_amd/csrc/tree.cuh
+++ b/alphazero_gym_amd/csrc/tree.cuh
@@ -97,6 +97,9 @@
     typedef IdT PoolId;
     Rec* hot; IdT* pool; float* prior;
     double* state;
+    double* lw; Warm* warm; int wm;
+    __device__ __forceinline__ int warm_slot(int id) const { return id == 0 ? 0 : 1 + (id & (wm > 0 ? wm - 1 : 0)); }
+    __device__ __forceinline__ bool warm_hit(int id, int nrec) const { return wm > 0 && (id == 0 || id + wm >= nrec); }
     __device__ __forceinline__ int child_at(int, const Rec& hp, int i, int) const {
         return hp.n_child == 1 ? (int)hp.first : (int)pool[4 * (int)hp.cbase + i];
     }
@@ -155,7 +158,7 @@
 __device__ __forceinline__ void clear_pad(RecM& h) { h.cbase = 0; }
 __device__ __forceinline__ void clear_pad(RecL& h) { h.pad = 0; }
 
-template <bool CONT, int TLDS, typename F, typename PW = int>
+template <bool CONT, int TLDS, typename F, typename PW = int, bool WARM = false>
 __device__ __forceinline__ void backup_from(const TreeStore<TLDS>& ts, const Cold* cold, double* edge_W, int j, float V, int sub,
                                             float gamma_f, double gamma, bool firstlvl, bool at_leaf, double Rv, F&& on_node,
                                             const PW* s_pw = nullptr, int pw_cap = 0) {
@@ -173,7 +176,10 @@
         Rec mrec = ts.hot[mine];
         const bool is_edge = (sub < cnt) && (mine != 0);
         double r = 0.0, W = 0.0;
-        if (is_edge) { r = cold[mine].r; W = edge_W[mine]; }
+        if (is_edge) {
+            r = cold[mine].r;
+            if constexpr (WARM) W = ts.lw[mine]; else W = edge_W[mine];
+        }
         double myR = 0.0;
         const int nedge = hit_root ? cnt - 1 : cnt;
 #pragma unroll 1
@@ -195,7 +201,7 @@
                 double Wn = W + myR;
                 mrec.Q = tree_div(Wn, (double)en);
                 mrec.edge_n = (decltype(mrec.edge_n))en;
-                edge_W[mine] = Wn;
+                if constexpr (WARM) ts.lw[mine] = Wn; else edge_W[mine] = Wn;
             }
             if (!(at_leaf && sub == 0)) {
                 mrec.node_n = (decltype(mrec.node_n))(mrec.node_n + 1);
@@ -214,7 +220,7 @@
     }
 }
 
-template <bool CONT, int TLDS, typename F, typename PW = int>
+template <bool CONT, int TLDS, typename F, typename PW = int, bool WARM = false>
 __device__ __forceinline__ void backup_path(const TreeStore<TLDS>& ts, const Cold* cold, double* edge_W, float V, int sub, float gamma_f,
                                             double gamma, int D, int my_depth, int pid, double pr, double& pW, F&& on_node,
                                             typename TreeStore<TLDS>::Rec& rec, double& chainR, bool same_chain = false,
@@ -275,7 +281,7 @@
             double Wn = pW + myR;
             rec.Q = tree_div(Wn, (double)en);
             rec.edge_n = (decltype(rec.edge_n))en;
-            edge_W[pid] = Wn;
+            if constexpr (WARM) ts.lw[pid] = Wn; else edge_W[pid] = Wn;
             pW = Wn;
         }
         if (my_depth < D) {
@@ -286,6 +292,6 @@
     }
     if (D >= 16) {
         int j = __shfl(par, (D - 15) & 15, 16);
-        backup_from<CONT, TLDS>(ts, cold, edge_W, j, V, sub, gamma_f, gamma, false, false, Rv, on_node, s_pw, pw_cap);
-    }
-}
+        backup_from<CONT, TLDS, F, PW, WARM>(ts, cold, edge_W, j, V, sub, gamma_f, gamma, false, false, Rv, on_node, s_pw, pw_cap);
+    }
+}
diff --git a/alphazero_gym_amd/csrc/tree_phases.cuh b/alphazero_gym_amd/csrc/tree_phases.cuh
--- a/alphazero_gym_amd/csrc/tree_phases.cuh
+++ b/alphazero_gym_amd/csrc/tree_phases.cuh
@@ -146,7 +146,7 @@
     return win;
 }
 
-template <int ENV, int TLDS, int TPW = 16, bool OBS8 = false>
+template <int ENV, int TLDS, int TPW = 16, bool OBS8 = false, bool WARM = false>
 __device__ __forceinline__ void tree_init_root(const KParams& P, TreeState& st, const TreeStore<TLDS>& ts, Cold* cold, double* edge_W,
                                                float* action, int tree, bool live, int sub, int tl, unsigned gtree, float* obsT) {
     constexpr bool CONT = EnvFamily<ENV>::CONT;
@@ -175,7 +175,14 @@
             if (CONT) c.s[2] = sn;
             c.r = 0.0; c.V = 0.0f; c.mu = 0.0f; c.sg = 0.0f; c.pad = 0.0f;
             cold[0] = c;
-            edge_W[0] = 0.0;
+            if constexpr (WARM) {
+                ts.lw[0] = 0.0;
+                Warm w;
+                w.s[0] = c.s[0]; w.s[1] = c.s[1]; w.s[2] = c.s[2]; w.mu = 0.0f; w.sg = 0.0f;
+                ts.warm[0] = w;
+            } else {
+                edge_W[0] = 0.0;
+            }
             if (CONT) action[0] = 0.0f;
             if constexpr (!CONT && TLDS != TS_GLOBAL) {
                 if (ts.state) {
@@ -193,7 +200,7 @@
         }
 }
 
-template <int ENV, int TLDS, bool GMM, int NCH, int PSTR = 64, bool RESUME = false, int SPEC = 0, typename PW = int>
+template <int ENV, int TLDS, bool GMM, int NCH, int PSTR = 64, bool RESUME = false, int SPEC = 0, typename PW = int, bool WARM = false>
 __device__ __forceinline__ void tree_phase_a(const KParams& P, TreeState& st, const TreeStore<TLDS>& ts, Cold* cold, double* edge_W,
                                              float* action, size_t tb, int sim, int sub, int tl, unsigned gtree, const f32x4* parts,
                                              const float* bhead, const double* s_sqrt STAMP_PARAM_OPT, const PW* s_pw = nullptr) {
@@ -223,6 +230,9 @@
                 sg = azg_expf(ls);
             }
             if (sub == 0) { cold[st.leaf].V = V; cold[st.leaf].mu = mu; cold[st.leaf].sg = sg; }
+            if constexpr (WARM) {
+                if (sub == 0) { Warm* w = ts.warm + ts.warm_slot(st.leaf); w->mu = mu; w->sg = sg; }
+            }
             if (sim < 0) {
                 int k = st.nrec++;
                 if constexpr (GMM) gmm_pick(gd, P.ncomp, P.seed, gtree, P.search_idx, (unsigned)k, &mu, &sg);
@@ -232,7 +242,7 @@
                     Rec h = make_edge<Rec>((double)V, 0);
                     clear_pad(h);
                     ts.hot[k] = h;
-                    edge_W[k] = 0.0;
+                    if constexpr (WARM) ts.lw[k] = 0.0; else edge_W[k] = 0.0;
                     action[k] = a;
                 }
                 ts.child_append(0, make_edge<Rec>(0.0, 0), 0, k, st.ptop, sub == 0, P.Kp,
@@ -296,8 +306,9 @@
         if (!TLDS) tree_fence();
         const bool keep = !CONT && Spec<SPEC, ENV>::plain(P);
         Rec myrec;
-        backup_path<CONT, TLDS>(ts, cold, edge_W, V, sub, P.gamma_f, P.gamma, st.path_D, st.my_depth, st.pid, st.pr, st.pW,
-                                [&](int pn) { if (keep) refresh_best<ENV, TLDS, SPEC>(P, ts, pn, sub, s_sqrt); }, myrec, st.chainR,
+        auto on_node = [&](int pn) { if (keep) refresh_best<ENV, TLDS, SPEC>(P, ts, pn, sub, s_sqrt); };
+        backup_path<CONT, TLDS, decltype(on_node)&, PW, WARM>(ts, cold, edge_W, V, sub, P.gamma_f, P.gamma, st.path_D, st.my_depth, st.pid, st.pr, st.pW,
+                                on_node, myrec, st.chainR,
                                 RESUME && !CONT && st.repeat,
                                 CONT ? 0.0 : discrete_env_reward(Spec<SPEC, ENV>::env(P)),
                                 CONT ? 0.0 : (st.need_eval ? discrete_env_reward(Spec<SPEC, ENV>::env(P)) : discrete_env_terminal_reward(Spec<SPEC, ENV>::env(P))),
@@ -341,7 +352,7 @@
     float cact;
 };
 
-template <int ENV, int TLDS, int SPEC, bool FETCH = false, typename PW = int>
+template <int ENV, int TLDS, int SPEC, bool FETCH = false, typename PW = int, bool WARM = false>
 __device__ __forceinline__ void tree_phase_b2(const KParams& P, TreeState& st, const TreeStore<TLDS>& ts, Cold* cold, double* edge_W, float* action,
                                               const BDeferred& d, int sub, unsigned gtree, const PW* s_pw) {
     typedef typename TreeStore<TLDS>::Rec Rec;
@@ -357,7 +368,7 @@
             clear_pad(h);
             set_wnext(h, P.pw0 > 0);
             ts.hot[d.chosen] = h;
-            edge_W[d.chosen] = 0.0;
+            if constexpr (WARM) ts.lw[d.chosen] = 0.0; else edge_W[d.chosen] = 0.0;
             action[d.chosen] = d.cact;
         }
         ts.child_append(d.p, hp, (int)hp.n_child, d.chosen, st.ptop, sub == 0, P.Kp,
@@ -380,11 +391,12 @@
     eps_prepare(P, st, gtree, sub);
 }
 
-template <int ENV, int TLDS, bool GMM, int TPW = 16, typename PW = int, bool FETCH = true, bool RESUME = false, int SPEC = 0, bool OBS8 = false, bool DEFER = false>
+template <int ENV, int TLDS, bool GMM, int TPW = 16, typename PW = int, bool FETCH = true, bool RESUME = false, int SPEC = 0, bool OBS8 = false, bool DEFER = false, bool WARM = false>
 __device__ __forceinline__ void tree_phase_b(const KParams& P, TreeState& st, const TreeStore<TLDS>& ts, Cold* cold, double* edge_W,
                                              float* action, size_t tb, int sub, int tl, unsigned gtree, const double* s_sqrt,
                                              const PW* s_pw, float* obsT STAMP_PARAM, BDeferred* def = nullptr) {
     static_assert(!DEFER || (ENV == AZG_ENV_PENDULUM_V1 && !GMM), "deferred expansion: Pendulum family, squashed-Normal head");
+    static_assert(!WARM || (DEFER && !FETCH && TLDS != TS_GLOBAL), "warm ring: the deferred-expansion kernels (the path's rewards fetched by the caller)");
     constexpr bool CONT = EnvFamily<ENV>::CONT;
     constexpr int S = CONT ? 2 : 4;
     typedef typename TreeStore<TLDS>::Rec Rec;
@@ -410,7 +422,9 @@
     Cold cp;
     bool from_cold = true;
     if constexpr (!CONT && TLDS != TS_GLOBAL) from_cold = (ts.state == nullptr);
-    if (from_cold) cp = cold[p];
+    Warm wp;
+    if constexpr (WARM) wp = ts.warm[0];
+    else if (from_cold) cp = cold[p];
     else { cp.s[0] = cp.s[1] = cp.s[2] = cp.s[3] = 0.0; }
     if (!resumed) { st.path_D = 0; st.my_depth = sub == 0 ? 0 : -1; st.pid = 0; }
     if (!keep_slot) { st.pr = 0.0; st.pW = 0.0; }
@@ -442,7 +456,9 @@
         STAMP_ADD(7, tl0, tl1);
         STAMP2(tl2, 8, 9);
         Cold cn;
-        if constexpr (CONT && EARLY_COLD) cn = cold[chosen];
+        [[maybe_unused]] Warm wn;
+        if constexpr (WARM) wn = ts.warm[ts.warm_slot(chosen)];
+        else if constexpr (CONT && EARLY_COLD) cn = cold[chosen];
         Rec hc = ts.hot[chosen];
         if (!(hc.flags & FLAG_EXPANDED)) break;
         STAMP2(tl3, 9, 10);
@@ -457,7 +473,8 @@
         if constexpr (EnvFamily<ENV>::TERM) {
             if (hc.flags & FLAG_TERMINAL) { hit_terminal = true; break; }
         }
-        if (CONT) { if constexpr (EARLY_COLD) cp = cn; else cp = cold[p]; }
+        if constexpr (WARM) wp = wn;
+        else if (CONT) { if constexpr (EARLY_COLD) cp = cn; else cp = cold[p]; }
         else if (from_cold) { cp.s[0] = cold[p].s[0]; cp.s[1] = cold[p].s[1]; cp.s[2] = cold[p].s[2]; cp.s[3] = cold[p].s[3]; }
         STAMP2(tl4, 10, 11);
         STAMP_ADD(8, tl0, tl2);
@@ -470,6 +487,16 @@
     }
     STAMP2(tb1, 13, 14);
     STAMP_ADD(13, tb0, tb1);
+    if constexpr (WARM) {
+        cp.s[0] = wp.s[0]; cp.s[1] = wp.s[1]; cp.s[2] = wp.s[2]; cp.mu = wp.mu; cp.sg = wp.sg;
+        if (!ts.warm_hit(p, st.nrec)) {
+            const Cold* c = cold + p;
+            double g0 = c->s[0], g1 = c->s[1], g2 = c->s[2];
+            float gm = c->mu, gs = c->sg;
+            asm volatile("" : "+v"(g0), "+v"(g1), "+v"(g2), "+v"(gm), "+v"(gs));
+            cp.s[0] = g0; cp.s[1] = g1; cp.s[2] = g2; cp.mu = gm; cp.sg = gs;
+        }
+    }
     if (hit_terminal) {
         st.leaf = p;
     } else {
@@ -504,7 +531,10 @@
         double ns[S], r, sn;
         int done;
         if (CONT) {
-            if (!widen) cact = action[chosen];
+            if (!widen) {
+                cact = action[chosen];
+                if constexpr (WARM) asm volatile("" : "+v"(cact));
+            }
             if constexpr (DEFER) {
                 pendulum_dynamics(Spec<SPEC, ENV>::v1(P), cp.s, cp.s[2], cact, ns);
                 r = 0.0; done = 0;
@@ -531,6 +561,9 @@
         if constexpr (DEFER) {
             def->pending = true; def->widen = widen; def->p = p; def->chosen = chosen; def->cact = cact;
             if (sub == 0) { cold[chosen].s[0] = ns[0]; cold[chosen].s[1] = ns[1]; cold[chosen].s[2] = sn; }
+            if constexpr (WARM) {
+                if (sub == 0) { Warm* w = ts.warm + ts.warm_slot(chosen); w->s[0] = ns[0]; w->s[1] = ns[1]; w->s[2] = sn; }
+            }
         } else if (sub == 0) {
             Cold c;
 #pragma unroll
```
